# NinV/Background-Debiased-Video-CIL

Measured on AMD Instinct MI355X. Metric: clips/sec fwd+bwd TSM-R50 8x224^2 bs32/GPU, higher is better.
Workload: dtype f32; 1 GPU; TSM-ResNet50 fwd+bwd+SGD step, synthetic 32x8x3x224x224 clips per GPU, 101 classes, SimpleLinear+CrossEntropyLoss, dropout 0.5, random-init weights; fp32 tensors, accumulators and results; conv products: fp32 via 3xbf16 split, 6 MFMA products, fp32 accumulate (dropped terms <= 2^-24 relative); conv_arith=bf16x3, clips_per_gpu=32, global_batch=32, parallelism=dp1

## Files before the change

background-debiased-video-cil_amd/_lib.py:

```python
from __future__ import annotations

import ctypes
import os
from ctypes import POINTER, Structure, c_char_p, c_float, c_int, c_int32, c_int64, c_size_t, c_uint16, c_uint64, c_void_p

_HERE = os.path.dirname(os.path.abspath(__file__))
_OVERRIDE = os.environ.get('BDVCIL_LIB_PATH')
LIB_PATH = _OVERRIDE or os.path.join(_HERE, 'csrc', 'libbdvcil_hip.so')
ABI_VERSION = 32

_lib = None


class ConvGeom(Structure):
    _fields_ = [(n, c_int32) for n in
                ('N', 'H', 'W', 'Cin', 'Ho', 'Wo', 'Cout', 'R', 'S', 'stride', 'pad', 'T', 'fold', 'pad_w', 'Rt', 'st_t', 'act_dtype')]

    def key(self):
        return tuple(getattr(self, n) for n, _ in self._fields_)


P = c_void_p
_F3 = c_float * 3


class ConvAffine(Structure):
    _fields_ = [('scale', c_void_p), ('shift', c_void_p), ('residual', c_void_p), ('relu', c_int32)]


class BnStatFuse(Structure):
    _fields_ = [('y', c_void_p), ('relu_mask', c_void_p), ('mean', c_void_p), ('invstd', c_void_p), ('partial', c_void_p),
                ('relu_scale', c_void_p), ('relu_shift', c_void_p)]

class JpegInfo(Structure):
    _fields_ = [('width', c_int32), ('height', c_int32), ('ncomp', c_int32), ('h', c_int32 * 3), ('v', c_int32 * 3),
                ('blocks_w', c_int32 * 3), ('blocks_h', c_int32 * 3), ('down_w', c_int32 * 3), ('down_h', c_int32 * 3),
                ('qt', (c_uint16 * 64) * 3), ('coef_offset', c_int64 * 3), ('coef_count', c_int64)]

    def geometry_key(self):
        return (self.width, self.height, self.ncomp, tuple(self.h), tuple(self.v))


SIGNATURES = {
    'bdv_last_error': (c_char_p, []),
    'bdv_abi_version': (c_int, []),
    'bdv_source_hash': (c_char_p, []),
    'bdv_conv_workspace_bytes': (c_size_t, [POINTER(ConvGeom), c_int]),
    'bdv_conv_fprop_stat_rows': (c_int, [POINTER(ConvGeom)]),
    'bdv_conv_fprop': (c_int, [P, P, P, POINTER(ConvGeom), P, POINTER(ConvAffine), P, c_size_t, P]),
    'bdv_conv_fprop_x3': (c_int, [P, P, P, POINTER(ConvGeom), P, POINTER(ConvAffine), P, c_size_t, P]),
    'bdv_conv_dgrad_stat_rows': (c_int, [POINTER(ConvGeom)]),
    'bdv_conv_dgrad': (c_int, [P, P, P, P, P, POINTER(ConvGeom), POINTER(BnStatFuse), P, c_size_t, P]),
    'bdv_conv_dgrad_x3': (c_int, [P, P, P, P, P, P, POINTER(ConvGeom), POINTER(BnStatFuse), P, c_size_t, P]),
    'bdv_conv_weight_planes_bytes': (c_size_t, [POINTER(ConvGeom)]),
    'bdv_conv_split_weights': (c_int, [P, POINTER(ConvGeom), P, P, P]),
    'bdv_conv_fprop_pre_ok': (c_int, [POINTER(ConvGeom)]),
    'bdv_conv_fprop_pre_stat_rows': (c_int, [POINTER(ConvGeom)]),
    'bdv_conv_wgrad_pre_ok': (c_int, [POINTER(ConvGeom)]),
    'bdv_conv_debug_force_tile': (c_int, [c_int]),
    'bdv_conv_uses_planes': (c_int, [POINTER(ConvGeom), c_int, c_int]),
    'bdv_conv_kernel_name': (c_int, [POINTER(ConvGeom), c_int, c_int, c_char_p, c_size_t]),
    'bdv_conv_fprop_pl_stat_rows': (c_int, [POINTER(ConvGeom), c_int]),
    'bdv_conv_dgrad_pl_stat_rows': (c_int, [POINTER(ConvGeom), c_int]),
    'bdv_conv_fprop_pl': (c_int, [P, P, P, P, POINTER(ConvGeom), P, POINTER(ConvAffine), P, c_size_t, c_int, P, P, P]),
    'bdv_conv_dgrad_pl': (c_int, [P, P, P, P, P, P, POINTER(ConvGeom), POINTER(BnStatFuse), P, c_size_t, c_int, P]),
    'bdv_conv_wgrad': (c_int, [P, P, P, c_float, POINTER(ConvGeom), P, c_size_t, P]),
    'bdv_conv_wgrad_splits': (c_int, [POINTER(ConvGeom)]),
    'bdv_conv_wgrad_partial': (c_int, [P, P, POINTER(ConvGeom), P, c_size_t, P]),
    'bdv_conv_wgrad_partial_x3': (c_int, [P, P, POINTER(ConvGeom), P, c_size_t, P]),
    'bdv_conv_wgrad_pl_splits': (c_int, [POINTER(ConvGeom)]),
    'bdv_conv_wgrad_partial_pl': (c_int, [P, P, POINTER(ConvGeom), P, c_size_t, c_int, P, P, P]),
    'bdv_wgrad_reduce_batched': (c_int, [P, P, P, P, c_int, c_float, P]),
    'bdv_bn_workspace_bytes': (c_size_t, [c_int64, c_int]),
    'bdv_bn_train_stats': (c_int, [P, c_int64, c_int, P, P, c_float, c_float, P, P, P, P, P, P, P, c_size_t, P]),
    'bdv_bn_train_finalize': (c_int, [P, c_int, c_int64, c_int, P, P, c_float, c_float, P, P, P, P, P, P, P]),
    'bdv_bn_eval_params': (c_int, [c_int, P, P, P, P, c_float, P, P, P]),
    'bdv_bn_apply': (c_int, [P, P, P, P, P, P, P, P, c_int64, c_int, c_int, c_int, P]),
    'bdv_bn_backward': (c_int, [P, P, P, P, P, P, P, P, P, c_float, c_int64, c_int, c_int, P, c_int, P, P, P, c_size_t, c_int, P]),
    'bdv_bn_finalize_scratch_bytes': (c_size_t, [c_int]),
    'bdv_bn_finalize_splits': (c_int, [c_int, c_int]),
    'bdv_bn_train_finalize_split': (c_int, [P, c_int, c_int64, c_int, P, P, c_float, c_float, P, P, P, P, P, P, c_int, P, c_size_t, P]),
    'bdv_bn_backward_split': (c_int, [P, P, P, P, P, P, P, P, P, c_float, c_int64, c_int, c_int, P, c_int, P, P, P, c_size_t, c_int,
                                      c_int, P, c_size_t, P]),
    'bdv_bn_pair_workspace_bytes': (c_size_t, [c_int64, c_int]),
    'bdv_bn_backward_pair': (c_int, [P, P, P, P, P, P, P, c_int, P, P, P, P, P, P, P, P, P, P, c_int64, c_int, P, c_size_t, c_int, c_int,
                                     P, c_size_t, P]),
    'bdv_bn_eval_backward': (c_int, [P, P, P, P, P, P, P, P, P, P, P, c_float, c_int64, c_int, P, c_size_t, c_int, c_int, P, c_size_t, P]),
    'bdv_bn_backward_maxpool_split': (c_int, [P, P, P, P, P, P, P, P, P, P, c_float, c_int, c_int, c_int, c_int, P, c_size_t, c_int,
                                              c_int, P, c_size_t, P]),
    'bdv_bn_backward_maxpool': (c_int, [P, P, P, P, P, P, P, P, P, P, c_float, c_int, c_int, c_int, c_int, P, c_size_t, c_int, P]),
    'bdv_relu_bwd': (c_int, [P, P, P, P, c_int64, c_int, P]),
    'bdv_add': (c_int, [P, P, P, c_int64, c_int, P]),
    'bdv_nchw3_to_nhwc4': (c_int, [P, P, c_int, c_int, c_int, P]),
    'bdv_maxpool_fwd': (c_int, [P, P, P, c_int, c_int, c_int, c_int, c_int, P]),
    'bdv_maxpool_bwd': (c_int, [P, P, P, c_int, c_int, c_int, c_int, c_int, P]),
    'bdv_maxpool_t2_fwd': (c_int, [P, P, P, c_int64, c_int64, P]),
    'bdv_maxpool_t2_bwd': (c_int, [P, P, P, c_int64, c_int64, P]),
    'bdv_bn_relu_maxpool_fwd': (c_int, [P, P, P, P, P, P, c_int, c_int, c_int, c_int, c_int, P]),
    'bdv_avgpool_fwd': (c_int, [P, P, c_int, c_int, c_int, c_int, P]),
    'bdv_avgpool_bwd': (c_int, [P, P, c_int, c_int, c_int, c_int, P]),
    'bdv_bgmix_normalize_u8': (c_int, [P, P, c_int, P, c_float, _F3, _F3, _F3, P, P, c_int, c_int, c_int, c_int, P]),
    'bdv_bg_resize_crop_u8': (c_int, [P, c_int, c_int, c_int, c_int, c_int, P, P, c_int, c_int, P, P]),
    'bdv_resize_linear_u8': (c_int, [P, c_int, c_int, c_int, P, c_int, P, P, c_int, c_int, P]),
    'bdv_jpeg_parse': (c_int, [P, c_size_t, POINTER(JpegInfo)]),
    'bdv_jpeg_entropy_decode': (c_int, [P, c_size_t, POINTER(JpegInfo), P]),
    'bdv_jpeg_entropy_decode_batch': (c_int, [P, P, c_int, POINTER(JpegInfo), P, P, c_int]),
    'bdv_jpeg_workspace_bytes': (c_size_t, [POINTER(JpegInfo), c_int]),
    'bdv_jpeg_reconstruct_u8': (c_int, [P, P, POINTER(JpegInfo), c_int, P, c_size_t, P, P]),
    'bdv_temporal_median_u8': (c_int, [P, c_int64, P, P, P, P, c_int, c_int, c_int, P, P]),
    'bdv_jpeg_encode_info': (c_int, [c_int, c_int, c_int, POINTER(JpegInfo)]),
    'bdv_jpeg_forward_u8': (c_int, [P, c_int, c_int, c_int, c_int, P, P]),
    'bdv_jpeg_encode_bound': (c_size_t, [c_int, c_int]),
    'bdv_jpeg_entropy_encode': (c_int, [P, c_int, c_int, c_int, P, c_size_t, P]),
    'bdv_jpeg_entropy_encode_batch': (c_int, [P, c_int, c_int, c_int, c_int, P, c_size_t, P, c_int]),
    'bdv_crop_normalize_u8': (c_int, [P, P, c_int, c_int, c_int, _F3, _F3, P, P, c_int, c_int, c_int, c_int, P]),
    'bdv_actor_cut_mix_u8': (c_int, [P, c_int, c_int, c_int, P, c_int, c_int, c_int, P, P, c_int64, c_int, c_int, c_int, c_int, _F3, _F3, P,
                                     c_int, P, P]),
    'bdv_lsc_fwd': (c_int, [P, P, P, P, P, P, c_int, c_int, c_int, c_int, P]),
    'bdv_lsc_bwd': (c_int, [P, P, P, P, P, P, P, P, c_float, P, c_int, c_int, c_int, c_int, P]),
    'bdv_linear_fwd': (c_int, [P, P, P, P, c_int, c_int, c_int, P]),
    'bdv_linear_bwd': (c_int, [P, P, P, P, P, P, c_float, c_int, c_int, c_int, P]),
    'bdv_consensus_fwd': (c_int, [P, P, c_int, c_int, c_int, P]),
    'bdv_consensus_bwd': (c_int, [P, P, c_int, c_int, c_int, P]),
    'bdv_dropout': (c_int, [P, P, c_int64, c_float, c_uint64, P]),
    'bdv_lsc_loss': (c_int, [P, P, P, c_float, c_int, P, P, P, P, c_int, c_int, P]),
    'bdv_softce_loss': (c_int, [P, P, P, P, P, c_int, c_int, P]),
    'bdv_icarl_targets': (c_int, [P, P, c_int, P, P, c_int, c_int, P]),
    'bdv_acm_targets': (c_int, [P, P, P, c_float, P, c_int, c_int, P]),
    'bdv_softmax_mean': (c_int, [P, P, c_int, c_int, c_int, c_int, P]),
    'bdv_topk_acc': (c_int, [P, P, P, c_int, c_int, P]),
    'bdv_repr_from_features': (c_int, [P, P, P, c_int, c_int, c_int, c_int, P]),
    'bdv_nme_workspace_bytes': (c_size_t, [c_int, c_int]),
    'bdv_nme_classify': (c_int, [P, P, P, P, c_int, c_int, c_int, c_int, P, c_size_t, P]),
    'bdv_class_means': (c_int, [P, P, P, c_int, c_int, c_int, P]),
    'bdv_herding_workspace_bytes': (c_size_t, [c_int, c_int]),
    'bdv_herding_select': (c_int, [P, c_int, c_int, c_int, c_int, P, P, P, P, c_size_t, P]),
    'bdv_randaug_workspace_bytes': (c_size_t, [c_int, c_int, c_int, c_int]),
    'bdv_randaug_apply': (c_int, [P, P, P, P, c_int, c_int, c_int, c_int, P, c_size_t, P]),
    'bdv_reduce_workspace_bytes': (c_size_t, []),
    'bdv_kd_mse_fwd': (c_int, [P, P, P, c_int64, P, c_size_t, c_int, P]),
    'bdv_kd_mse_bwd': (c_int, [P, P, P, c_float, P, c_int64, c_int, P]),
    'bdv_multi_sqnorm': (c_int, [P, P, c_int, P, P, c_size_t, P]),
    'bdv_clip_coef': (c_int, [P, c_float, c_float, P, P]),
    'bdv_multi_sgd': (c_int, [P, P, P, P, P, P, c_int, c_float, c_float, P, P]),
}


class HipExtensionError(RuntimeError):
# ... 47 lines not shown
```

background-debiased-video-cil_amd/csrc/conv_mfma.hip:

```cpp
#include <stdlib.h>
#include "common.h"

#ifdef BDV_STAMPS
__device__ unsigned long long* g_stamp_buf = nullptr;
__device__ int g_stamp_cap = 0;
#define BDV_STAMP(slot)                                                                                                          \
  do {                                                                                                                           \
    if (threadIdx.x == 0 && g_stamp_buf != nullptr && (int)(blockIdx.x + gridDim.x * blockIdx.y) < g_stamp_cap) {                 \
      unsigned long long* q_ = g_stamp_buf + (size_t)(blockIdx.x + gridDim.x * blockIdx.y) * 8;                                  \
      if ((slot) == 4) asm volatile("s_waitcnt vmcnt(0)" ::: "memory");                                                          \
      q_[slot] = __builtin_amdgcn_s_memtime();                                                                                   \
      if ((slot) == 0) { q_[5] = __builtin_amdgcn_s_memrealtime(); q_[7] = __builtin_amdgcn_s_getreg((4 << 0) | (0 << 6) | (31 << 11)); } \
      if ((slot) == 4) q_[6] = __builtin_amdgcn_s_memrealtime();                                                                 \
    }                                                                                                                            \
  } while (0)
#else
#define BDV_STAMP(slot) do { } while (0)
#endif

namespace {

constexpr int BK = 32;

struct Geom {
// ... 43 lines not shown
}

__device__ __forceinline__ void fast_divmod(int m, int d, float rcp, int& q, int& r) {
  q = (int)((float)m * rcp);
  r = m - q * d;
  if (r < 0) {
    r += d;
    --q;
  }
  if (r >= d) {
    r -= d;
    ++q;
  }
}

template <int LDA, int LDB, int TM, int TN, int MS, int NS, bool SWA, bool SWB>
__device__ __forceinline__ void mma_stage(const float* __restrict__ As, const float* __restrict__ Bs,
                                          f32x16 (&acc)[TM][TN], int wm0, int wn0, int lane) {
  const int r = lane & 31, h = lane >> 5;
  const float* apv[SWA ? 8 : 1];
  const float* bpv[SWB ? 8 : 1];
#pragma unroll
  for (int c = 0; c < (SWA ? 8 : 1); ++c) apv[c] = As + h * LDA + wm0 + (r ^ (4 * c));
#pragma unroll
  for (int c = 0; c < (SWB ? 8 : 1); ++c) bpv[c] = Bs + h * LDB + wn0 + (r ^ (4 * c));
  auto ap = [&](int s, int i) { return apv[SWA ? ((s >> 1) & 7) : 0][2 * s * LDA + MS * i]; };
  auto bp = [&](int s, int j) { return bpv[SWB ? ((s >> 1) & 7) : 0][2 * s * LDB + NS * j]; };
  float a[2][TM], b[2][TN];
#pragma unroll
  for (int i = 0; i < TM; ++i) a[0][i] = ap(0, i);
#pragma unroll
  for (int j = 0; j < TN; ++j) b[0][j] = bp(0, j);
#pragma unroll
  for (int s = 0; s < BK / 2; ++s) {
    const int cur = s & 1, nxt = cur ^ 1;
    if (s + 1 < BK / 2) {
#pragma unroll
      for (int i = 0; i < TM; ++i) a[nxt][i] = ap(s + 1, i);
#pragma unroll
      for (int j = 0; j < TN; ++j) b[nxt][j] = bp(s + 1, j);
    }
#pragma unroll
    for (int i = 0; i < TM; ++i)
#pragma unroll
      for (int j = 0; j < TN; ++j)
        acc[i][j] = __builtin_amdgcn_mfma_f32_32x32x2f32(a[cur][i], b[cur][j], acc[i][j], 0, 0, 0);
    __builtin_amdgcn_sched_group_barrier(0x100, TM + TN, 0);
    __builtin_amdgcn_sched_group_barrier(0x008, TM * TN, 0);
  }
}

__device__ __forceinline__ int shift_class(int c, int fold) {
  return (fold > 0) ? (c < fold ? 1 : (c < 2 * fold ? -1 : 0)) : 0;
}

template <int LD, int PASSES>
__device__ __forceinline__ void store_transposed(float* __restrict__ dst, const float4 (&v)[PASSES], int tid) {
  const int row = tid >> 3, kg = tid & 7;
#pragma unroll
  for (int p = 0; p < PASSES; ++p) {
    float* d = dst + (4 * kg) * LD + ((row + 32 * p) ^ (4 * kg));
    d[0] = v[p].x;
    d[LD] = v[p].y;
    d[2 * LD] = v[p].z;
    d[3 * LD] = v[p].w;
  }
}

template <int LD, int COLS, int PASSES>
__device__ __forceinline__ void store_direct(float* __restrict__ dst, const float4 (&v)[PASSES], int tid) {
  constexpr int V = COLS / 4;
#pragma unroll
  for (int p = 0; p < PASSES; ++p) {
    const int idx = tid + 256 * p;
    const int krow = idx / V, c4 = idx - krow * V;
    *reinterpret_cast<float4*>(dst + krow * LD + 4 * c4) = v[p];
  }
}

__device__ __forceinline__ int acc_row(int reg, int lane) { return (reg & 3) + 8 * (reg >> 2) + 4 * (lane >> 5); }

struct Work {
  int dp_tiles, rem_tiles, split;
};

__device__ __forceinline__ int xcd_remap(int b, int n) {
  const int q = n >> 3, r = n & 7, x = b & 7, j = b >> 3;
  return (x < r ? x * (q + 1) : r * (q + 1) + (x - r) * q) + j;
}

struct WorkItem {
  int tile, kb, ke, pslot;
};

__device__ __forceinline__ WorkItem get_work(int b, const Work& wk, int nk) {
  WorkItem it;
  if (b < wk.dp_tiles) {
    it.tile = xcd_remap(b, wk.dp_tiles);
    it.kb = 0;
    it.ke = nk;
    it.pslot = -1;
  } else {
    const int rem = b - wk.dp_tiles;
    const int rt = rem / wk.split, sl = rem - rt * wk.split;
    it.tile = wk.dp_tiles + rt;
    it.kb = (int)(((long long)sl * nk) / wk.split);
    it.ke = (int)(((long long)(sl + 1) * nk) / wk.split);
    it.pslot = wk.split > 1 ? rem : -1;
  }
  return it;
}

template <int TM, int TN, int NT = 256>
__device__ __forceinline__ void store_partial(float* __restrict__ slab, int pslot, const f32x16 (&acc)[TM][TN], int tid) {
  float* base = slab + (size_t)pslot * (TM * TN * 16) * NT + tid;
#pragma unroll
  for (int i = 0; i < TM; ++i)
#pragma unroll
    for (int j = 0; j < TN; ++j)
#pragma unroll
      for (int e = 0; e < 16; ++e) base[(size_t)((i * TN + j) * 16 + e) * NT] = acc[i][j][e];
}

template <int TM, int TN>
__device__ __forceinline__ void zero_acc(f32x16 (&acc)[TM][TN]) {
#pragma unroll
  for (int i = 0; i < TM; ++i)
#pragma unroll
    for (int j = 0; j < TN; ++j)
#pragma unroll
      for (int e = 0; e < 16; ++e) acc[i][j][e] = 0.f;
}

__device__ __forceinline__ void fprop_store(float* __restrict__ y, const Geom& g, int row, int col, float v) {
  if (row < g.M) y[(size_t)row * g.Cout + col] = v;
}

struct BnStat {
  const void* y;
  const uint32_t* mask;
  const float* mean;
  const float* invstd;
  float* partial;
  int MT;
  const float* rscale;
  const float* rshift;
};

struct StatAcc {
  float4 s1, s2, mu, is;
  __device__ __forceinline__ void init(const BnStat& st, int col) {
    s1 = s2 = make_float4(0.f, 0.f, 0.f, 0.f);
    mu = *reinterpret_cast<const float4*>(st.mean + col);
    is = *reinterpret_cast<const float4*>(st.invstd + col);
  }
  __device__ __forceinline__ static unsigned sign_bits(const BnStat& st, int col, const float4 yv) {
    const float4 rsc = *reinterpret_cast<const float4*>(st.rscale + col), rsh = *reinterpret_cast<const float4*>(st.rshift + col);
    return (fmaf(yv.x, rsc.x, rsh.x) > 0.f ? 1u : 0u) | (fmaf(yv.y, rsc.y, rsh.y) > 0.f ? 2u : 0u) |
           (fmaf(yv.z, rsc.z, rsh.z) > 0.f ? 4u : 0u) | (fmaf(yv.w, rsc.w, rsh.w) > 0.f ? 8u : 0u);
  }
  __device__ __forceinline__ void accumulate(const float4 v, const float4 yv) {
    s1.x += v.x; s1.y += v.y; s1.z += v.z; s1.w += v.w;
    s2.x += v.x * ((yv.x - mu.x) * is.x);
    s2.y += v.y * ((yv.y - mu.y) * is.y);
    s2.z += v.z * ((yv.z - mu.z) * is.z);
    s2.w += v.w * ((yv.w - mu.w) * is.w);
  }
};

template <int BN, int NT = 256>
__device__ __forceinline__ void stat_flush(const StatAcc& a, const BnStat& st, float* __restrict__ smem, int Cin, int mt, int nt,
                                           int tid) {
  constexpr int V = BN / 4, G = NT / V;
  __syncthreads();
  const int grp = tid / V, c4 = tid - grp * V;
  *reinterpret_cast<float4*>(smem + grp * BN + 4 * c4) = a.s1;
  *reinterpret_cast<float4*>(smem + (G + grp) * BN + 4 * c4) = a.s2;
  __syncthreads();
  if (tid < BN) {
    float x = 0.f, y = 0.f;
#pragma unroll
    for (int k = 0; k < G; ++k) {
      x += smem[k * BN + tid];
      y += smem[(G + k) * BN + tid];
    }
    st.partial[(size_t)mt * Cin + nt * BN + tid] = x;
    st.partial[((size_t)st.MT + mt) * Cin + nt * BN + tid] = y;
  }
}

template <int BM, int BN, int WM, int WN, class F>
__device__ __forceinline__ void staged_epilogue(const f32x16 (&acc)[BM / WM / 32][BN / WN / 32], float* __restrict__ smem, int tid,
                                                F&& emit) {
  constexpr int TM = BM / WM / 32, TN = BN / WN / 32;
  constexpr int NT = 64 * WM * WN;
  constexpr int V = BN / 4;
  constexpr int PER = WM * 32 * V / NT;
  const int lane = tid & 63, wave = tid >> 6;
  const int wm = wave / WN, wn0 = (wave % WN) * 32;
#pragma unroll
  for (int i = 0; i < TM; ++i) {
    __syncthreads();
#pragma unroll
    for (int j = 0; j < TN; ++j)
#pragma unroll
      for (int e = 0; e < 16; ++e) smem[(wm * 32 + acc_row(e, lane)) * BN + wn0 + 32 * WN * j + (lane & 31)] = acc[i][j][e];
    __syncthreads();
#pragma unroll
    for (int q = 0; q < PER; ++q) {
      const int idx = tid + NT * q;
      const int lr = idx / V, c4 = idx - lr * V;
      const float4 v = *reinterpret_cast<const float4*>(smem + lr * BN + 4 * c4);
      emit(32 * WM * i + lr, 4 * c4, v);
    }
// ... 636 lines not shown
  f32x16 acc[TM][TN];
  zero_acc<TM, TN>(acc);
  const int nk = (g.Ktot + BK - 1) / BK;
  load(0);
  for (int kt = 0; kt < nk; ++kt) {
    __syncthreads();
    store_transposed<LDA, AP>(As, ra, tid);
    store_transposed<LDB, BP>(Bs, rb, tid);
    __syncthreads();
    if (kt + 1 < nk) load(kt + 1);
    mma_stage<LDA, LDB, TM, TN, 32 * WM, 32 * WN, true, true>(As, Bs, acc, wm0, wn0, lane);
  }
  fprop_epilogue<BM, BN, WM, WN>(acc, smem, y, g, epi, mt, nt, tid);
}

template <int BM, int BN, int WM, int WN>
__global__ __launch_bounds__(256, 2) void conv_fprop_c4_x3_kernel(const float* __restrict__ x, const float* __restrict__ w,
                                                                   float* __restrict__ y, Geom g, int NT, FpropEpi epi) {
  constexpr int TM = BM / WM / 32, TN = BN / WN / 32;
  constexpr int AP = BM / 32, BP = BN / 32;
  static_assert(3 * (BM + BN) * X3_LDK * 2 >= WM * 32 * BN * 4, "the epilogue stages a tile pass in the same LDS");
  __shared__ __attribute__((aligned(16))) unsigned short smem16[3 * (BM + BN) * X3_LDK];
  unsigned short* const As = smem16;
  unsigned short* const Bs = smem16 + 3 * BM * X3_LDK;
  float* const smem = reinterpret_cast<float*>(smem16);
  const int tile = xcd_remap(blockIdx.x, epi.MT * NT);
  const int mt = tile / NT, nt = tile - mt * NT;
  const int tid = threadIdx.x;
  const int lane = tid & 63, wave = tid >> 6;
  const int wm0 = (wave / WN) * 32, wn0 = (wave % WN) * 32;
  const int arow = tid >> 3, kg = tid & 7;
  const int HoWo = g.Ho * g.Wo;
  const int RS = g.R * g.S, RST = RS * g.Rt;
  const int Tin = g.T * g.st_t, pad_t = g.Rt / 2;
  const __amdgpu_buffer_rsrc_t xr = __builtin_amdgcn_make_buffer_rsrc((void*)x, 0, g.N * g.st_t * g.H * g.W * 16, 0x00020000);
  const __amdgpu_buffer_rsrc_t wr = __builtin_amdgcn_make_buffer_rsrc((void*)w, 0, g.Cout * g.Ktot * 4, 0x00020000);

  int a_base[AP], a_hi0[AP], a_wi0[AP], a_t0[AP];
#pragma unroll
  for (int p = 0; p < AP; ++p) {
    const int m = mt * BM + arow + 32 * p;
    const bool ok = m < g.M;
    const int mm = ok ? m : 0;
    const int n = mm / HoWo;
    const int rem = mm - n * HoWo;
    const int ho = rem / g.Wo, wo = rem - ho * g.Wo;
    a_hi0[p] = ok ? ho * g.stride - g.pad : -(1 << 20);
    a_wi0[p] = wo * g.stride - g.pad_w;
    a_t0[p] = (n % g.T) * g.st_t - pad_t;
    a_base[p] = (((n * g.st_t - pad_t) * g.H + ho * g.stride - g.pad) * g.W + wo * g.stride - g.pad_w) * 16;
  }
  float4 ra[AP], rb[BP];
  auto load = [&](int kt) {
    const int tap = kt * (BK / 4) + kg;
    int dt, rs, r, s;
    fast_divmod(tap, RS, g.rcp_RS, dt, rs);
    fast_divmod(rs, g.S, g.rcp_S, r, s);
    const bool kv = tap < RST;
#pragma unroll
    for (int p = 0; p < AP; ++p) {
      const bool v = kv && (unsigned)(a_hi0[p] + r) < (unsigned)g.H && (unsigned)(a_wi0[p] + s) < (unsigned)g.W &&
                     (unsigned)(a_t0[p] + dt) < (unsigned)Tin;
      ra[p] = buf_load16(xr, (a_base[p] + ((dt * g.H + r) * g.W + s) * 16) | (v ? 0 : kOOB), 0);
    }
#pragma unroll
    for (int p = 0; p < BP; ++p)
      rb[p] = buf_load16(wr, (((nt * BN + arow + 32 * p) * g.Ktot + tap * 4) * 4) | (kv ? 0 : kOOB), 0);
  };
  f32x16 acc[TM][TN];
  zero_acc<TM, TN>(acc);
  const int nk = (g.Ktot + BK - 1) / BK;
  load(0);
  for (int kt = 0; kt < nk; ++kt) {
    __syncthreads();
    store_split3<BM, AP>(As, ra, tid);
    store_split3<BN, BP>(Bs, rb, tid);
    __syncthreads();
    if (kt + 1 < nk) load(kt + 1);
    mma_stage_x3<TM, TN, 32 * WM, 32 * WN, BM, BN>(As, Bs, acc, wm0, wn0, lane);
  }
  fprop_epilogue<BM, BN, WM, WN>(acc, smem, y, g, epi, mt, nt, tid);
}

template <int BM, int BN, int WM, int WN>
__global__ __launch_bounds__(64 * WM * WN) void conv_fprop_fixup_kernel(const float* __restrict__ slab, float* __restrict__ y, Geom g,
                                                                int NT, Work wk, FpropEpi epi) {
  constexpr int TM = BM / WM / 32, TN = BN / WN / 32;
  constexpr int NACC = TM * TN * 16;
  constexpr int NTHR = 64 * WM * WN;
  __shared__ __attribute__((aligned(16))) float smem[WM * 32 * BN];
  const int rt = blockIdx.x, tile = wk.dp_tiles + rt;
  const int mt = tile / NT, nt = tile - mt * NT;
  const int tid = threadIdx.x;
  f32x16 acc[TM][TN];
  zero_acc<TM, TN>(acc);
  for (int sl = 0; sl < wk.split; ++sl) {
    const float* src = slab + (size_t)(rt * wk.split + sl) * NACC * NTHR + tid;
#pragma unroll
    for (int i = 0; i < TM; ++i)
#pragma unroll
      for (int j = 0; j < TN; ++j)
#pragma unroll
        for (int e = 0; e < 16; ++e) acc[i][j][e] += src[(size_t)((i * TN + j) * 16 + e) * NTHR];
  }
  fprop_epilogue<BM, BN, WM, WN>(acc, smem, y, g, epi, mt, nt, tid);
}

template <int BM, int BN, int WM, int WN>
__global__ __launch_bounds__(256, 3) void conv_dgrad_kernel(const float* __restrict__ dy, const float* __restrict__ w,
                                                          float* __restrict__ dx, const float* __restrict__ add_src,
                                                          const uint32_t* __restrict__ add_mask, Geom g, int NT, Work wk,
                                                          float* __restrict__ slab, BnStat stat) {
  constexpr int LDA = BM, LDB = BN;
  constexpr int TM = BM / WM / 32, TN = BN / WN / 32;
  constexpr int AP = BM / 32, BP = BN / 32;
  constexpr int BV = BN / 4;
  constexpr int AOFF = (BK * LDA + 3) & ~3;
  constexpr int SMEM = (AOFF + BK * LDB) > (WM * 32 * BN) ? (AOFF + BK * LDB) : (WM * 32 * BN);
  __shared__ __attribute__((aligned(16))) float smem[SMEM];
  float* const As = smem;
  float* const Bs = smem + AOFF;

  const int st = g.stride;
  const int ph = blockIdx.y / st, pw = blockIdx.y - ph * st;
  const int Hc = (g.H - ph + st - 1) / st, Wc = (g.W - pw + st - 1) / st;
  const int Mc = g.N * Hc * Wc;
  const int MT = (Mc + BM - 1) / BM;
  const int r0 = (ph + g.pad) % st, s0 = (pw + g.pad_w) % st;
  const int nr = r0 < g.R ? (g.R - r0 + st - 1) / st : 0;
  const int ns = s0 < g.S ? (g.S - s0 + st - 1) / st : 0;
  const int bh = (ph + g.pad - r0) / st, bw = (pw + g.pad_w - s0) / st;
  const int ntap = nr * ns;
  const int nk = ntap * g.Cout / BK;

  int mt, nt;
  WorkItem it;
  if (st == 1) {
    it = get_work(blockIdx.x, wk, nk);
    mt = it.tile / NT;
    nt = it.tile - mt * NT;
  } else {
    const int id = blockIdx.x;
    const int xcd = id & 7, jj = id >> 3;
    mt = (jj / NT) * 8 + xcd;
    nt = jj % NT;
    if (mt >= MT) return;
    it.tile = 0;
    it.kb = 0;
    it.ke = nk;
    it.pslot = -1;
  }

  const int tid = threadIdx.x;
  const int lane = tid & 63, wave = tid >> 6;
  const int wm0 = (wave / WN) * 32, wn0 = (wave % WN) * 32;
  const int arow = tid >> 3, kg = tid & 7;
  const int HcWc = Hc * Wc;
  const int RS = g.R * g.S;
  const __amdgpu_buffer_rsrc_t yr = __builtin_amdgcn_make_buffer_rsrc((void*)dy, 0, g.N * g.Ho * g.Wo * g.Cout * 4, 0x00020000);
  const __amdgpu_buffer_rsrc_t wr = __builtin_amdgcn_make_buffer_rsrc((void*)w, 0, g.Cout * RS * g.Cin * 4, 0x00020000);

  int a_base[AP], a_h[AP], a_w[AP];
#pragma unroll
  for (int p = 0; p < AP; ++p) {
    const int m = mt * BM + arow + 32 * p;
    const bool ok = m < Mc;
    const int mm = ok ? m : 0;
    const int n = mm / HcWc;
    const int rem = mm - n * HcWc;
    const int hc = rem / Wc, wc = rem - hc * Wc;
    a_h[p] = ok ? hc + bh : -(1 << 20);
    a_w[p] = wc + bw;
    a_base[p] = ((n * g.Ho + hc + bh) * g.Wo + wc + bw) * g.Cout * 4 + 16 * kg;
  }
  int b_base[BP];
#pragma unroll
  for (int p = 0; p < BP; ++p) {
    const int idx = tid + 256 * p;
    const int krow = idx / BV, c4 = idx - krow * BV;
    b_base[p] = (krow * RS * g.Cin + nt * BN + 4 * c4) * 4;
  }

  int chunk = ntap > 0 ? it.kb / ntap : 0, ir, is;
  {
    const int ct = ntap > 0 ? it.kb - chunk * ntap : 0;
    ir = ns > 0 ? ct / ns : 0;
// ... 115 lines not shown
    const int rem = mm - n * HcWc;
    const int hc = rem / Wc, wc = rem - hc * Wc;
    a_h[p] = ok ? hc + bh : -(1 << 20);
    a_w[p] = wc + bw;
    a_base[p] = ((n * g.Ho + hc + bh) * g.Wo + wc + bw) * g.Cout * 4 + 16 * kg;
  }
  int b_base[BP];
#pragma unroll
  for (int p = 0; p < BP; ++p) b_base[p] = ((nt * BN + arow + 32 * p) * g.Cout + 4 * kg) * 4;

  int chunk = ntap > 0 ? it.kb / ntap : 0, ir, is;
  {
    const int ct = ntap > 0 ? it.kb - chunk * ntap : 0;
    ir = ns > 0 ? ct / ns : 0;
    is = ct - ir * ns;
  }

  float4 ra[AP], rb[BP];
  u32x4 rbp[BPRE ? 3 * BQ : 1];
  auto load = [&]() {
    const int tap = (r0 + ir * st) * g.S + (s0 + is * st);
    const int koff_a = (chunk * BK - (ir * g.Wo + is) * g.Cout) * 4;
    const int koff_b = (tap * g.Cin * g.Cout + chunk * BK) * 4;
#pragma unroll
    for (int p = 0; p < AP; ++p) {
      const bool v = (unsigned)(a_h[p] - ir) < (unsigned)g.Ho && (unsigned)(a_w[p] - is) < (unsigned)g.Wo;
      ra[p] = buf_load16(yr, (a_base[p] + koff_a) | (v ? 0 : kOOB), 0);
    }
    if (BPRE) {
#pragma unroll
      for (int pl = 0; pl < 3; ++pl)
#pragma unroll
        for (int q = 0; q < BQ; ++q)
          rbp[pl * BQ + q] = __builtin_amdgcn_raw_buffer_load_b128(wr, (nt * BN + brow + 64 * q) * 64 + 16 * bc + pl * plane_bytes,
                                                                   (tap * nchunk + chunk) * g.Cin * 64, 0);
    } else {
#pragma unroll
      for (int p = 0; p < BP; ++p) rb[p] = buf_load16(wr, b_base[p], koff_b);
    }
    is += 1;
    const int w1 = (is == ns) ? 1 : 0;
    is = w1 ? 0 : is;
    ir += w1;
    const int w2 = (ir == nr) ? 1 : 0;
    ir = w2 ? 0 : ir;
    chunk += w2;
  };

  f32x16 acc[TM][TN];
  zero_acc<TM, TN>(acc);

  if (it.ke > it.kb) {
    load();
    for (int kt = it.kb; kt < it.ke; ++kt) {
      __syncthreads();
      store_split3<BM, AP>(As, ra, tid);
      if (BPRE) {
#pragma unroll
        for (int pl = 0; pl < 3; ++pl)
#pragma unroll
          for (int q = 0; q < BQ; ++q) *reinterpret_cast<u32x4*>(Bs + (pl * BN + brow + 64 * q) * X3_LDK + 8 * bc) = rbp[pl * BQ + q];
      } else {
        store_split3<BN, BP>(Bs, rb, tid);
      }
      __syncthreads();
      if (kt + 1 < it.ke) load();
      mma_stage_x3<TM, TN, 32 * WM, 32 * WN, BM, BN>(As, Bs, acc, wm0, wn0, lane);
    }
  }
  if (it.pslot >= 0) {
    store_partial<TM, TN>(slab, it.pslot, acc, tid);
    return;
  }

  dgrad_epilogue<BM, BN, WM, WN, true, 4, true>(acc, smem, tid, dx, add_src, add_mask, g, mt, nt, Mc, stat, [&](int mrow) {
    if (st == 1) return mrow;
    const int n = mrow / HcWc;
    const int rem = mrow - n * HcWc;
    const int hc = rem / Wc;
    return (n * g.H + hc * st + ph) * g.W + (rem - hc * Wc) * st + pw;
  });
}

template <int BM, int BN, int WM, int WN>
__global__ __launch_bounds__(64 * WM * WN) void conv_dgrad_fixup_kernel(const float* __restrict__ slab, float* __restrict__ dx,
                                                                const float* __restrict__ add_src,
                                                                const uint32_t* __restrict__ add_mask, Geom g, int NT, Work wk,
                                                                BnStat stat) {
  constexpr int TM = BM / WM / 32, TN = BN / WN / 32;
  constexpr int NACC = TM * TN * 16;
  constexpr int NTHR = 64 * WM * WN;
  __shared__ __attribute__((aligned(16))) float smem[WM * 32 * BN];
  const int rt = blockIdx.x, tile = wk.dp_tiles + rt;
  const int mt = tile / NT, nt = tile - mt * NT;
  const int tid = threadIdx.x;
  f32x16 acc[TM][TN];
  zero_acc<TM, TN>(acc);
  for (int sl = 0; sl < wk.split; ++sl) {
    const float* src = slab + (size_t)(rt * wk.split + sl) * NACC * NTHR + tid;
#pragma unroll
    for (int i = 0; i < TM; ++i)
#pragma unroll
      for (int j = 0; j < TN; ++j)
#pragma unroll
        for (int e = 0; e < 16; ++e) acc[i][j][e] += src[(size_t)((i * TN + j) * 16 + e) * NTHR];
  }
  dgrad_epilogue<BM, BN, WM, WN>(acc, smem, tid, dx, add_src, add_mask, g, mt, nt, g.M, stat, [](int mrow) { return mrow; });
}

template <int BM, int BN, int WM, int WN, bool C4, bool INCR>
__global__ __launch_bounds__(256, 3) void conv_wgrad_kernel(const float* __restrict__ dy, const float* __restrict__ x,
                                                          float* __restrict__ slab, Geom g, int MTw, int NTw,
                                                          int kt_per_split) {
  constexpr int LDA = BM, LDB = BN;
  constexpr int TM = BM / WM / 32, TN = BN / WN / 32;
  constexpr int AP = BM / 32, BP = BN / 32;
  constexpr int AV = BM / 4, BV = BN / 4;
  __shared__ __attribute__((aligned(16))) float smem[BK * (LDA + LDB)];
  float* const As = smem;
  float* const Bs = smem + BK * LDA;

  const int tiles = MTw * NTw;
  const int wi = xcd_remap(blockIdx.x, gridDim.x);
  const int split = wi / tiles;
  const int tile = wi - split * tiles;
  const int mt = tile % MTw, nt = tile / MTw;
  const int tid = threadIdx.x;
  const int lane = tid & 63, wave = tid >> 6;
  const int wm0 = (wave / WN) * 32, wn0 = (wave % WN) * 32;
  const int HoWo = g.Ho * g.Wo;
  const int frame_bytes = g.H * g.W * g.Cin * 4;
  const __amdgpu_buffer_rsrc_t xr = __builtin_amdgcn_make_buffer_rsrc((void*)x, 0, g.N * frame_bytes, 0x00020000);
  const __amdgpu_buffer_rsrc_t yr = __builtin_amdgcn_make_buffer_rsrc((void*)dy, 0, g.M * g.Cout * 4, 0x00020000);

  int a_off[AP];
#pragma unroll
  for (int p = 0; p < AP; ++p) {
    const int idx = tid + 256 * p;
    const int krow = idx / AV, c4 = idx - krow * AV;
    a_off[p] = (krow * g.Cout + mt * BM + 4 * c4) * 4;
  }
  int b_krow[BP], b_off[BP], b_r[BP], b_s[BP], b_cls[BP];
  bool b_cok[BP];
#pragma unroll
  for (int p = 0; p < BP; ++p) {
    const int idx = tid + 256 * p;
    const int krow = idx / BV, c4 = idx - krow * BV;
    b_krow[p] = krow;
    int tap, ci;
    if (C4) {
      const int ncol = nt * BN + 4 * c4;
      tap = ncol / g.Cin;
      ci = ncol - tap * g.Cin;
      b_cok[p] = ncol < g.Ktot;
    } else {
      const int per_tap = g.Cin / BN;
      tap = nt / per_tap;
      ci = (nt - tap * per_tap) * BN + 4 * c4;
      b_cok[p] = true;
    }
    b_r[p] = tap / g.S - g.pad;
    b_s[p] = tap % g.S - g.pad_w;
    b_cls[p] = shift_class(ci, g.fold);
    b_off[p] = ((b_r[p] * g.W + b_s[p]) * g.Cin + ci) * 4 + b_cls[p] * frame_bytes;
  }

  const int kt_begin = split * kt_per_split;
  const int nkt_all = (g.M + BK - 1) / BK;
  const int kt_end = min(kt_begin + kt_per_split, nkt_all);

  const int st = g.stride;
  const int d_ho = BK / g.Wo, d_wo = BK - d_ho * g.Wo;
  const int wrap_w = g.Wo * st, wrap_h = g.Ho * st;
  const int px = g.Cin * 4;
  const int inc0 = (d_ho * st * g.W + d_wo * st) * px;
  const int inc1 = (st * g.W - wrap_w) * px;
  const int inc2 = (g.H * g.W - wrap_h * g.W) * px;
  int s_hi[BP], s_wi[BP], s_t[BP], s_off[BP];
  if (INCR) {
#pragma unroll
    for (int p = 0; p < BP; ++p) {
      const int m = split * kt_per_split * BK + b_krow[p];
      const int n = m / HoWo;
      const int rem = m - n * HoWo;
      const int ho = rem / g.Wo, wo = rem - ho * g.Wo;
      s_hi[p] = ho * st;
      s_wi[p] = wo * st;
      s_t[p] = n % g.T;
// ... 372 lines not shown
  const int tx = threadIdx.x & 31, ty = threadIdx.x >> 5;
  const size_t plane = (size_t)Cout * RS * Cin;
#pragma unroll
  for (int p = 0; p < 4; ++p) {
    const int co_l = ty + 8 * p;
    const float a = w[((size_t)(co0 + co_l) * RS + tap) * Cin + ci0 + tx];
    const __bf16 hi = (__bf16)a;
    const float r1 = a - (float)hi;
    const __bf16 mid = (__bf16)r1;
    const __bf16 lo = (__bf16)(r1 - (float)mid);
    const unsigned short h16 = __builtin_bit_cast(unsigned short, hi), m16 = __builtin_bit_cast(unsigned short, mid),
                         l16 = __builtin_bit_cast(unsigned short, lo);
    if (F != nullptr) {
      const size_t o = (((size_t)(ci0 >> 5) * RS + tap) * Cout + co0 + co_l) * 32 + tx;
      F[o] = h16;
      F[plane + o] = m16;
      F[2 * plane + o] = l16;
    }
    tile[0][co_l][tx] = h16;
    tile[1][co_l][tx] = m16;
    tile[2][co_l][tx] = l16;
  }
  if (D == nullptr) return;
  __syncthreads();
#pragma unroll
  for (int p = 0; p < 4; ++p) {
    const int ci_l = ty + 8 * p;
    const size_t o = (((size_t)tap * (Cout >> 5) + (co0 >> 5)) * Cin + ci0 + ci_l) * 32 + tx;
    D[o] = tile[0][tx][ci_l];
    D[plane + o] = tile[1][tx][ci_l];
    D[2 * plane + o] = tile[2][tx][ci_l];
  }
}

using PlSet0 = std::integral_constant<int, 0>;
using PlSet1 = std::integral_constant<int, 1>;
template <typename LoadF, typename StoreF, typename MmaF>
__device__ __forceinline__ void pl_pipeline2(int n, LoadF&& load, StoreF&& store, MmaF&& mma, bool late = false) {
  load(PlSet0{});
  store(0, PlSet0{});
  if (n > 1) load(PlSet1{});
  if (n > 2) load(PlSet0{});
  __syncthreads();
  BDV_STAMP(1);
  int i = 0;
  if (late) {
    for (; i + 4 < n; i += 2) {
      store(1, PlSet1{});
      load(PlSet1{});
      mma(0);
      __syncthreads();
      store(0, PlSet0{});
      load(PlSet0{});
      mma(1);
      __syncthreads();
    }
  } else {
    for (; i + 4 < n; i += 2) {
      mma(0);
      store(1, PlSet1{});
      load(PlSet1{});
      __syncthreads();
      mma(1);
      store(0, PlSet0{});
      load(PlSet0{});
      __syncthreads();
    }
  }
  for (; i < n; i += 2) {
    mma(0);
    if (i + 1 < n) store(1, PlSet1{});
    if (i + 3 < n) load(PlSet1{});
    __syncthreads();
    if (i + 1 >= n) break;
    mma(1);
    if (i + 2 < n) store(0, PlSet0{});
    if (i + 4 < n) load(PlSet0{});
    __syncthreads();
  }
}

constexpr int pl_waves_per_simd(int waves, int np, bool fits128) { return np == 1 && waves == 8 && fits128 ? 4 : waves == 4 ? 2 : waves / 4; }

template <int BM, int BN, int WM, int WN, int NBUF, int NP = 3, bool PRE = false, int ES = 4>
__global__ __launch_bounds__(64 * WM * WN, pl_waves_per_simd(WM * WN, NP, BN == 64 || (BM == 128 && BN == 256))) void conv_fprop_pl_kernel(const void* __restrict__ x,
                                                                                      const unsigned short* __restrict__ wp,
                                                                                      void* __restrict__ y, Geom g, int NT, Work wk,
                                                                                      float* __restrict__ slab, FpropEpi epi) {
  constexpr int NTHR = 64 * WM * WN;
  constexpr int TM = BM / WM / 32, TN = BN / WN / 32;
  constexpr int KG = ES == 2 ? 4 : 8;
  constexpr int AP = BM * KG / NTHR;
  constexpr int BPP = (BN * 4 + NTHR - 1) / NTHR;
  constexpr int PA = BM * 64, PB = BN * 64, STAGE = NP * (PA + PB);
  constexpr int SMEM = NBUF * STAGE >= WM * 32 * BN * 4 ? NBUF * STAGE : WM * 32 * BN * 4;
  static_assert(AP >= 1 && SMEM <= 160 * 1024, "tile / epilogue staging do not fit");
  __shared__ __attribute__((aligned(16))) unsigned char smem_b[SMEM];
  float* const smem = reinterpret_cast<float*>(smem_b);

  BDV_STAMP(0);
  const int nk = g.Ktot / BK;
  const WorkItem it = get_work(blockIdx.x, wk, nk);
  const int mt = it.tile / NT, nt = it.tile - mt * NT;

  const int tid = threadIdx.x;
  const int lane = tid & 63, wave = tid >> 6;
  const int wm = wave / WN, wn = wave % WN;
  const int arow = tid / KG, kg = tid % KG;
  const int brow = tid >> 2, bc = tid & 3;
  const int HoWo = g.Ho * g.Wo;
  static_assert(ES == 4 || (NP == 1 && !PRE), "bf16 storage: single-product arithmetic only");
  const int frame_bytes = g.H * g.W * g.Cin * ES;
  const int plane_bytes = g.Cout * g.Ktot * 2;

  const __amdgpu_buffer_rsrc_t xr = __builtin_amdgcn_make_buffer_rsrc((void*)x, 0, g.N * frame_bytes, 0x00020000);
  const __amdgpu_buffer_rsrc_t wr = __builtin_amdgcn_make_buffer_rsrc((void*)wp, 0, 3 * plane_bytes, 0x00020000);

  int a_base[AP], a_t[AP], a_hi0[AP], a_wi0[AP];
#pragma unroll
  for (int p = 0; p < AP; ++p) {
    const int m = mt * BM + arow + (NTHR / KG) * p;
    const bool ok = m < g.M;
    int n, rem, ho, wo;
    fast_divmod(ok ? m : 0, HoWo, g.rcp_HoWo, n, rem);
    fast_divmod(rem, g.Wo, g.rcp_Wo, ho, wo);
    a_t[p] = n % g.T;
    a_hi0[p] = ok ? ho * g.stride - g.pad : -(1 << 20);
    a_wi0[p] = wo * g.stride - g.pad_w;
    a_base[p] = ((n * g.H + ho * g.stride - g.pad) * g.W + wo * g.stride - g.pad_w) * g.Cin * ES + 16 * kg;
  }
  int b_base[BPP];
  const bool b_active = BN * 4 >= NTHR || tid < BN * 4;
#pragma unroll
  for (int q = 0; q < BPP; ++q) b_base[q] = b_active ? (nt * BN + brow + (NTHR / 4) * q) * 64 + 16 * bc : kOOB;

  const int RS = g.R * g.S;
  int chunk = it.kb / RS, r, s, kt_w = it.kb;
  {
    const int tap = it.kb - chunk * RS;
    r = tap / g.S;
    s = tap - r * g.S;
  }

  constexpr int NSET = NBUF;
  float4 ra[NSET][AP];
  u32x4 rb[NSET][NP * BPP];
  float4 psc[PRE ? NSET : 1], psh[PRE ? NSET : 1];
  unsigned pvalid[PRE ? NSET : 1];
  auto load = [&](auto set) __attribute__((always_inline)) {
    constexpr int SET = decltype(set)::value;
    if constexpr (PRE) {
      psc[SET] = *reinterpret_cast<const float4*>(epi.pre_scale + chunk * BK + 4 * kg);
      psh[SET] = *reinterpret_cast<const float4*>(epi.pre_shift + chunk * BK + 4 * kg);
      pvalid[SET] = 0u;
    }
    const int cls = shift_class(chunk * BK + (BK / KG) * kg, g.fold);
    const int koff_a = ((r * g.W + s) * g.Cin + chunk * BK) * ES;
    const int koff_b = kt_w * g.Cout * 64;
#pragma unroll
    for (int p = 0; p < AP; ++p) {
      const bool v = (unsigned)(a_hi0[p] + r) < (unsigned)g.H && (unsigned)(a_wi0[p] + s) < (unsigned)g.W &&
                     (unsigned)(a_t[p] + cls) < (unsigned)g.T;
      ra[SET][p] = buf_load16(xr, (a_base[p] + koff_a + cls * frame_bytes) | (v ? 0 : kOOB), 0);
      if constexpr (PRE) pvalid[SET] |= (v ? 1u : 0u) << p;
    }
#pragma unroll
    for (int pl = 0; pl < NP; ++pl)
#pragma unroll
      for (int q = 0; q < BPP; ++q) rb[SET][pl * BPP + q] = __builtin_amdgcn_raw_buffer_load_b128(wr, b_base[q] + pl * plane_bytes, koff_b, 0);
    kt_w += 1;
    s += 1;
    const int ws_ = (s == g.S) ? 1 : 0;
    s = ws_ ? 0 : s;
    r += ws_;
    const int wr_ = (r == g.R) ? 1 : 0;
    r = wr_ ? 0 : r;
    chunk += wr_;
  };
  const int st_a = ES == 2 ? pl_off(arow, kg) : pl_off(arow, kg >> 1) + 8 * (kg & 1), st_b = pl_off(brow, bc);
  const int fa[2] = {pl_frag_off(32 * wm, 0, lane), pl_frag_off(32 * wm, 1, lane)};
  const int fb[2] = {pl_frag_off(32 * wn, 0, lane), pl_frag_off(32 * wn, 1, lane)};
  auto store = [&](int stage, auto set) __attribute__((always_inline)) {
    constexpr int SET = decltype(set)::value;
    unsigned char* const As = smem_b + stage * STAGE;
    unsigned char* const Bs = As + NP * PA;
#pragma unroll
    for (int p = 0; p < AP; ++p) {
      float4 v = ra[SET][p];
      if constexpr (PRE) {
        const bool ok = (pvalid[SET] >> p) & 1u;
        v.x = ok ? fmaxf(fmaf(v.x, psc[SET].x, psh[SET].x), 0.f) : 0.f;
        v.y = ok ? fmaxf(fmaf(v.y, psc[SET].y, psh[SET].y), 0.f) : 0.f;
        v.z = ok ? fmaxf(fmaf(v.z, psc[SET].z, psh[SET].z), 0.f) : 0.f;
        v.w = ok ? fmaxf(fmaf(v.w, psc[SET].w, psh[SET].w), 0.f) : 0.f;
      }
      if constexpr (ES == 2) *reinterpret_cast<float4*>(As + st_a + (NTHR / KG) * p * 64) = v;
      else pl_split_store_at<NP>(As + st_a + (NTHR / KG) * p * 64, PA, v);
    }
    if (b_active) {
#pragma unroll
      for (int pl = 0; pl < NP; ++pl)
#pragma unroll
        for (int q = 0; q < BPP; ++q) *reinterpret_cast<u32x4*>(Bs + st_b + (pl * PB + (NTHR / 4) * q * 64)) = rb[SET][pl * BPP + q];
    }
  };
  f32x16 acc[TM][TN];
  zero_acc<TM, TN>(acc);

  if constexpr (NBUF == 2) {
    pl_pipeline2(it.ke - it.kb, load, store, [&](int stage) __attribute__((always_inline)) {
      mma_stage_pl<BM, BN, WM, WN, NP>(smem_b + stage * STAGE, smem_b + stage * STAGE + NP * PA, acc, fa, fb);
    }, g.stagger != 0 && wave >= WM * WN / 2);
  } else {
    load(PlSet0{});
    for (int kt = it.kb; kt < it.ke; ++kt) {
      __syncthreads();
      store(0, PlSet0{});
      __syncthreads();
      if (kt == it.kb) BDV_STAMP(1);
      if (kt + 1 < it.ke) load(PlSet0{});
      mma_stage_pl<BM, BN, WM, WN, NP>(smem_b, smem_b + NP * PA, acc, fa, fb);
    }
  }
  BDV_STAMP(2);

  if (it.pslot >= 0) {
    store_partial<TM, TN, NTHR>(slab, it.pslot, acc, tid);
    return;
  }
  fprop_epilogue<BM, BN, WM, WN, ES>(acc, smem, y, g, epi, mt, nt, tid);
  BDV_STAMP(3);
  BDV_STAMP(4);
}

template <int BM, int BN, int WM, int WN, int NBUF, int NP = 3, int ES = 4>
__global__ __launch_bounds__(64 * WM * WN, BM == 64 ? 4 : pl_waves_per_simd(WM * WN, NP, BN == 64)) void conv_dgrad_pl_kernel(const void* __restrict__ dy,
                                                                                      const unsigned short* __restrict__ dp,
                                                                                      void* __restrict__ dx,
                                                                                      const void* __restrict__ add_src,
                                                                                      const uint32_t* __restrict__ add_mask, Geom g,
                                                                                      int NT, Work wk, float* __restrict__ slab,
                                                                                      BnStat stat) {
  constexpr int NTHR = 64 * WM * WN;
  constexpr int TM = BM / WM / 32, TN = BN / WN / 32;
  constexpr int KG = ES == 2 ? 4 : 8;
  constexpr int AP = BM * KG / NTHR;
  constexpr int BPP = (BN * 4 + NTHR - 1) / NTHR;
  constexpr int PA = BM * 64, PB = BN * 64, STAGE = NP * (PA + PB);
  constexpr int SMEM = NBUF * STAGE >= WM * 32 * BN * 4 ? NBUF * STAGE : WM * 32 * BN * 4;
  static_assert(AP >= 1 && SMEM <= 160 * 1024, "tile / epilogue staging do not fit");
  __shared__ __attribute__((aligned(16))) unsigned char smem_b[SMEM];
  float* const smem = reinterpret_cast<float*>(smem_b);

  BDV_STAMP(0);
  const int st = g.stride;
  const int ph = blockIdx.y / st, pw = blockIdx.y - ph * st;
  const int Hc = (g.H - ph + st - 1) / st, Wc = (g.W - pw + st - 1) / st;
  const int Mc = g.N * Hc * Wc;
  const int MT = (Mc + BM - 1) / BM;
  const int r0 = (ph + g.pad) % st, s0 = (pw + g.pad_w) % st;
  const int nr = r0 < g.R ? (g.R - r0 + st - 1) / st : 0;
  const int ns = s0 < g.S ? (g.S - s0 + st - 1) / st : 0;
  const int bh = (ph + g.pad - r0) / st, bw = (pw + g.pad_w - s0) / st;
  const int ntap = nr * ns;
  const int nk = ntap * g.Cout / BK;

  int mt, nt;
  WorkItem it;
  if (st == 1) {
    it = get_work(blockIdx.x, wk, nk);
    mt = it.tile / NT;
    nt = it.tile - mt * NT;
  } else {
    const int id = blockIdx.x;
    const int xcd = id & 7, jj = id >> 3;
    mt = (jj / NT) * 8 + xcd;
    nt = jj % NT;
    if (mt >= MT) return;
    it.tile = 0;
    it.kb = 0;
    it.ke = nk;
    it.pslot = -1;
  }

  const int tid = threadIdx.x;
  const int lane = tid & 63, wave = tid >> 6;
  const int wm = wave / WN, wn = wave % WN;
  const int arow = tid / KG, kg = tid % KG;
  const int brow = tid >> 2, bc = tid & 3;
  const int HcWc = Hc * Wc;
  const int RS = g.R * g.S;
  const int plane_bytes = g.Cout * RS * g.Cin * 2;
  const __amdgpu_buffer_rsrc_t yr = __builtin_amdgcn_make_buffer_rsrc((void*)dy, 0, g.N * g.Ho * g.Wo * g.Cout * ES, 0x00020000);
  const __amdgpu_buffer_rsrc_t wr = __builtin_amdgcn_make_buffer_rsrc((void*)dp, 0, 3 * plane_bytes, 0x00020000);

  int a_base[AP], a_h[AP], a_w[AP];
#pragma unroll
  for (int p = 0; p < AP; ++p) {
    const int m = mt * BM + arow + (NTHR / KG) * p;
    const bool ok = m < Mc;
    const int mm = ok ? m : 0;
    const int n = mm / HcWc;
    const int rem = mm - n * HcWc;
    const int hc = rem / Wc, wc = rem - hc * Wc;
    a_h[p] = ok ? hc + bh : -(1 << 20);
    a_w[p] = wc + bw;
    a_base[p] = ((n * g.Ho + hc + bh) * g.Wo + wc + bw) * g.Cout * ES + 16 * kg;
  }
  int b_base[BPP];
  const bool b_active = BN * 4 >= NTHR || tid < BN * 4;
#pragma unroll
  for (int q = 0; q < BPP; ++q) b_base[q] = b_active ? (nt * BN + brow + (NTHR / 4) * q) * 64 + 16 * bc : kOOB;

  int chunk = ntap > 0 ? it.kb / ntap : 0, ir, is;
  {
    const int ct = ntap > 0 ? it.kb - chunk * ntap : 0;
    ir = ns > 0 ? ct / ns : 0;
    is = ct - ir * ns;
  }
  const int nchunk = g.Cout / BK;

  constexpr int NSET = NBUF;
  float4 ra[NSET][AP];
  u32x4 rb[NSET][NP * BPP];
  auto load = [&](auto set) __attribute__((always_inline)) {
    constexpr int SET = decltype(set)::value;
    const int tap = (r0 + ir * st) * g.S + (s0 + is * st);
    const int koff_a = (chunk * BK - (ir * g.Wo + is) * g.Cout) * ES;
    const int koff_b = (tap * nchunk + chunk) * g.Cin * 64;
#pragma unroll
    for (int p = 0; p < AP; ++p) {
      const bool v = (unsigned)(a_h[p] - ir) < (unsigned)g.Ho && (unsigned)(a_w[p] - is) < (unsigned)g.Wo;
      ra[SET][p] = buf_load16(yr, (a_base[p] + koff_a) | (v ? 0 : kOOB), 0);
    }
#pragma unroll
    for (int pl = 0; pl < NP; ++pl)
#pragma unroll
      for (int q = 0; q < BPP; ++q) rb[SET][pl * BPP + q] = __builtin_amdgcn_raw_buffer_load_b128(wr, b_base[q] + pl * plane_bytes, koff_b, 0);
    is += 1;
    const int w1 = (is == ns) ? 1 : 0;
    is = w1 ? 0 : is;
    ir += w1;
    const int w2 = (ir == nr) ? 1 : 0;
    ir = w2 ? 0 : ir;
    chunk += w2;
  };
  const int st_a = ES == 2 ? pl_off(arow, kg) : pl_off(arow, kg >> 1) + 8 * (kg & 1), st_b = pl_off(brow, bc);
  const int fa[2] = {pl_frag_off(32 * wm, 0, lane), pl_frag_off(32 * wm, 1, lane)};
  const int fb[2] = {pl_frag_off(32 * wn, 0, lane), pl_frag_off(32 * wn, 1, lane)};
  auto store = [&](int stage, auto set) __attribute__((always_inline)) {
    constexpr int SET = decltype(set)::value;
    unsigned char* const As = smem_b + stage * STAGE;
    unsigned char* const Bs = As + NP * PA;
#pragma unroll
    for (int p = 0; p < AP; ++p) {
      if constexpr (ES == 2) *reinterpret_cast<float4*>(As + st_a + (NTHR / KG) * p * 64) = ra[SET][p];
      else pl_split_store_at<NP>(As + st_a + (NTHR / KG) * p * 64, PA, ra[SET][p]);
    }
    if (b_active) {
#pragma unroll
      for (int pl = 0; pl < NP; ++pl)
#pragma unroll
        for (int q = 0; q < BPP; ++q) *reinterpret_cast<u32x4*>(Bs + st_b + (pl * PB + (NTHR / 4) * q * 64)) = rb[SET][pl * BPP + q];
    }
  };

  f32x16 acc[TM][TN];
  zero_acc<TM, TN>(acc);

  if (it.ke > it.kb) {
    if constexpr (NBUF == 2) {
      pl_pipeline2(it.ke - it.kb, load, store, [&](int stage) __attribute__((always_inline)) {
        mma_stage_pl<BM, BN, WM, WN, NP>(smem_b + stage * STAGE, smem_b + stage * STAGE + NP * PA, acc, fa, fb);
      }, g.stagger != 0 && wave >= WM * WN / 2);
    } else {
      load(PlSet0{});
      for (int kt = it.kb; kt < it.ke; ++kt) {
        __syncthreads();
        store(0, PlSet0{});
        __syncthreads();
        if (kt == it.kb) BDV_STAMP(1);
        if (kt + 1 < it.ke) load(PlSet0{});
        mma_stage_pl<BM, BN, WM, WN, NP>(smem_b, smem_b + NP * PA, acc, fa, fb);
      }
    }
  }
  BDV_STAMP(2);
  if (it.pslot >= 0) {
    store_partial<TM, TN, NTHR>(slab, it.pslot, acc, tid);
    return;
  }
  constexpr bool EPI_PIPE = TM * TN <= 4 && NP >= 2 && BM != 64;
  dgrad_epilogue<BM, BN, WM, WN, true, ES, EPI_PIPE>(acc, smem, tid, dx, add_src, add_mask, g, mt, nt, Mc, stat, [&](int mrow) {
    if (st == 1) return mrow;
    const int n = mrow / HcWc;
    const int rem = mrow - n * HcWc;
    const int hc = rem / Wc;
    return (n * g.H + hc * st + ph) * g.W + (rem - hc * Wc) * st + pw;
  });
  BDV_STAMP(3);
  BDV_STAMP(4);
}

typedef short s16x4_t __attribute__((ext_vector_type(4)));

template <int COLS, int NP = 3, int ROWS = 32>
__device__ __forceinline__ void pl_store_rows(unsigned char* __restrict__ base, int krow, int c4, const float4 v) {
  constexpr int PITCH = 2 * COLS + 64, PLANE = ROWS * PITCH;
  if constexpr (NP == 1) {
    *reinterpret_cast<u32x2_t*>(base + krow * PITCH + 8 * c4) = bf16_hi_pairs(v);
    return;
  }
  u32x2_t hi, mid, lo;
  split3_pairs(v, hi, mid, lo);
  unsigned char* q = base + krow * PITCH + 8 * c4;
  *reinterpret_cast<u32x2_t*>(q) = hi;
  *reinterpret_cast<u32x2_t*>(q + PLANE) = mid;
  if constexpr (NP == 3) *reinterpret_cast<u32x2_t*>(q + 2 * PLANE) = lo;
}

template <int COLS>
__device__ __forceinline__ bf16x8_t pl_frag_tr(const unsigned char* __restrict__ plane, int cb, int s, int lane) {
  constexpr int PITCH = 2 * COLS + 64;
  const int h = lane >> 5, q = (lane & 15) >> 2;
  const unsigned char* a = plane + (16 * s + 8 * h + q) * PITCH + 2 * (cb + 16 * ((lane >> 4) & 1) + 4 * (lane & 3));
  typedef __attribute__((address_space(3))) s16x4_t* lds_ptr;
  const s16x4_t lo4 = __builtin_amdgcn_ds_read_tr16_b64_v4i16((lds_ptr)(a));
  const s16x4_t hi4 = __builtin_amdgcn_ds_read_tr16_b64_v4i16((lds_ptr)(a + 4 * PITCH));
  typedef short s16x8_t __attribute__((ext_vector_type(8)));
  const s16x8_t f = __builtin_shufflevector(lo4, hi4, 0, 1, 2, 3, 4, 5, 6, 7);
  return __builtin_bit_cast(bf16x8_t, f);
}

template <int BM, int BN, int WM, int WN, bool INCR, int NP = 3, bool MTAP = false, int KW = 32, int ES = 4>
__global__ __launch_bounds__(64 * WM * WN, 2) void conv_wgrad_pl_kernel(const void* __restrict__ dy, const void* __restrict__ x,
                                                                         float* __restrict__ slab, Geom g, int MTw, int NTw,
                                                                         int kt_per_split, const float* __restrict__ pre_scale,
                                                                         const float* __restrict__ pre_shift) {
  constexpr int NTHR = 64 * WM * WN;
  constexpr int TM = BM / WM / 32, TN = BN / WN / 32;
  constexpr int GV = ES == 2 ? 8 : 4;
  static_assert(TM >= 1 && TN >= 1 && (32 * (BM / GV)) % NTHR == 0 && (32 * (BN / GV)) % NTHR == 0, "tile / thread mapping");
  static_assert(ES == 4 || NP == 1, "bf16 storage: single-product arithmetic (and Cin % 8 == 0: a 16-byte unit stays inside a filter tap)");
  constexpr int AV = BM / GV, BV = BN / GV;
  static_assert(KW == 32 || KW == 16, "pixels per stage");
  constexpr int NST = 32 / KW;
  constexpr int AP = KW * AV / NTHR, BP = KW * BV / NTHR;
  static_assert(AP >= 1 && BP >= 1 && (KW * AV) % NTHR == 0 && (KW * BV) % NTHR == 0, "stage / thread mapping");
  constexpr int PITCH_A = 2 * BM + 64, PITCH_B = 2 * BN + 64;
  constexpr int PLANE_A = KW * PITCH_A, PLANE_B = KW * PITCH_B;
  constexpr int STAGE = 3 * (PLANE_A + PLANE_B);
  __shared__ __attribute__((aligned(16))) unsigned char smem_b[NST * STAGE];
  __shared__ __attribute__((aligned(16))) float pre_lds[2][BN];
  const bool pre = pre_scale != nullptr;

  const int tiles = MTw * NTw;
  const int wi = xcd_remap(blockIdx.x, gridDim.x);
  const int split = wi / tiles;
  const int tile = wi - split * tiles;
  const int mt = tile % MTw, nt = tile / MTw;
  const int tid = threadIdx.x;
  const int lane = tid & 63, wave = tid >> 6;
  const int wm = wave / WN, wn = wave % WN;
  const int HoWo = g.Ho * g.Wo;
  const int frame_bytes = g.H * g.W * g.Cin * ES;
  const __amdgpu_buffer_rsrc_t xr = __builtin_amdgcn_make_buffer_rsrc((void*)x, 0, g.N * g.st_t * frame_bytes, 0x00020000);
  const __amdgpu_buffer_rsrc_t yr = __builtin_amdgcn_make_buffer_rsrc((void*)dy, 0, g.M * g.Cout * ES, 0x00020000);

  int a_off[AP], a_krow[AP];
#pragma unroll
  for (int p = 0; p < AP; ++p) {
    const int idx = tid + NTHR * p;
    a_krow[p] = idx / AV;
    a_off[p] = (a_krow[p] * g.Cout + mt * BM + GV * (idx % AV)) * ES;
  }
  int b_krow[BP], b_off[BP], b_cls[BP], b_r[BP], b_s[BP];
// ... 293 lines not shown
  p.nk = (g.Ktot + BK - 1) / BK;
  p.seg_bytes = (size_t)(p.wide ? 64 : 32) * 256 * sizeof(float);
  if (g.Cin % BK != 0) {
    p.wk.dp_tiles = p.MT * p.NT;
    p.wk.rem_tiles = 0;
    p.wk.split = 1;
  } else {
    p.wk = (x3 && p.wide) ? plan_work(p.MT * p.NT, p.nk, 0.9, p.seg_bytes, ws_bytes, 2)
                          : plan_work(p.MT * p.NT, p.nk, p.wide ? 1.7 : 0.85, p.seg_bytes, ws_bytes);
  }
  return p;
}

FdPlan plan_dgrad(const Geom& g, size_t ws_bytes, bool x3 = false) {
  FdPlan p;
  p.wide = (g.Cin % 128) == 0;
  const int bn = p.wide ? 128 : 64;
  const int st = g.stride;
  const int Mc0 = g.N * ((g.H + st - 1) / st) * ((g.W + st - 1) / st);
  p.MT = (Mc0 + 127) / 128;
  p.NT = g.Cin / bn;
  p.nk = g.R * g.S * g.Cout / BK;
  p.seg_bytes = (size_t)(p.wide ? 64 : 32) * 256 * sizeof(float);
  if (st == 1) {
    p.wk = (x3 && p.wide) ? plan_work(p.MT * p.NT, p.nk, 0.9, p.seg_bytes, ws_bytes, 2)
                          : plan_work(p.MT * p.NT, p.nk, p.wide ? 1.7 : 0.85, p.seg_bytes, ws_bytes);
  } else {
    p.wk.dp_tiles = ((p.MT + 7) / 8) * 8 * p.NT;
    p.wk.rem_tiles = 0;
    p.wk.split = 1;
  }
  return p;
}

struct PlCfg {
  int BM, BN, nbuf;
  double iter_us;
};
constexpr int kNumPlCfg = 6;
constexpr PlCfg kPlCfg[kNumPlCfg] = {{128, 256, 2, 2.7}, {256, 128, 2, 2.7}, {256, 256, 1, 4.7}, {256, 64, 2, 1.9}, {64, 128, 1, 0.7},
                                     {128, 128, 1, 1.6}};
constexpr int pl_cfg_wm(int cfg) { return cfg == 0 || cfg == 2 || cfg == 4 || cfg == 5 ? 2 : 4; }
constexpr int pl_cfg_wn(int cfg) { return cfg == 4 || cfg == 5 ? 2 : 8 / pl_cfg_wm(cfg); }
constexpr int pl_cfg_round(int cfg) { return cfg == 5 ? 512 : 256; }

struct PlPlan {
  int cfg;
  int MT, NT, nk;
  size_t seg_bytes;
  Work wk;
  double est_us;
};

Work plan_work_pl(int tiles, int nk, double iter_us, size_t seg_bytes, size_t ws_bytes, double* est_us, int W = 256) {
  Work wk;
  const int q = tiles / W, r = tiles - q * W;
  wk.dp_tiles = tiles;
  wk.rem_tiles = 0;
  wk.split = 1;
  double best = (double)(q + (r > 0 ? 1 : 0)) * nk * iter_us;
  if (r > 0 && nk >= 4) {
    for (int sp = 2; sp <= 16 && nk / sp >= 2; ++sp) {
      const size_t need = (size_t)r * sp * seg_bytes;
      if (need > ws_bytes) break;
      const int rounds = (r * sp + W - 1) / W;
      const int per = (nk + sp - 1) / sp;
      const double cost = ((double)q * nk + (double)rounds * per) * iter_us + 8.0 + 2.0 * (double)need / 4.0e6;
      if (cost < best * 0.97) {
        best = cost;
        wk.dp_tiles = q * W;
        wk.rem_tiles = r;
        wk.split = sp;
      }
    }
  }
  *est_us = best;
  return wk;
}

int g_pl_tile_forced = -2;
int pl_tile_override() {
  if (g_pl_tile_forced == -2) g_pl_tile_forced = getenv("BDVCIL_PL_TILE") ? atoi(getenv("BDVCIL_PL_TILE")) : -1;
  return g_pl_tile_forced;
}

int pl_pick(bool dgrad, int ncols, int nk, int taps, int stride, int pieces = 3, bool shifted = false) {
  const int forced = pl_tile_override();
  if (pieces == 1) {
    const bool small_ok = dgrad && stride == 1;
    if (forced >= 0 && forced < kNumPlCfg && ncols % kPlCfg[forced].BN == 0 && (forced != 4 || small_ok)) return forced;
    static const bool np1_small = getenv("BDVCIL_NP1_SMALL_TILES") == nullptr || atoi(getenv("BDVCIL_NP1_SMALL_TILES")) != 0;
    if (np1_small && small_ok && ncols % 128 == 0) return 4;
    return ncols % 256 == 0 ? 0 : ncols % 128 == 0 ? 1 : ncols % 64 == 0 ? 3 : -1;
  }
  if (pieces == 2) {
    if (forced >= 0 && forced < kNumPlCfg && ncols % kPlCfg[forced].BN == 0 && (forced != 4 || (dgrad && stride == 1))) return forced;
    const int c = pl_pick(dgrad, ncols, nk, taps, stride, 3, shifted);
    return c >= 0 ? c : ncols % 128 == 0 ? 5 : ncols % 64 == 0 ? 3 : -1;
  }
  if (forced == kNumPlCfg) return -1;
  if (forced >= 0 && ncols % kPlCfg[forced].BN == 0 && (forced != 4 || (dgrad && stride == 1))) return forced;
  if (ncols % 64 != 0) return -1;
  if (ncols % 128 != 0) return taps > 1 ? 3 : -1;
  if (!dgrad) {
    if (ncols % 256 != 0) return nk >= 16 ? 1 : -1;
    if (nk >= 16 || nk <= 2) return 0;
    return -1;
  }
  static const bool small_tiles = getenv("BDVCIL_DGRAD_64X128") != nullptr && atoi(getenv("BDVCIL_DGRAD_64X128")) == 1;
  if (ncols % 256 != 0) return taps > 1 && stride == 1 ? 1 : (small_tiles && taps == 1 && stride == 1 && nk >= 16 ? 4 : -1);
  if (stride == 2 && taps > 1) return 0;
  if (small_tiles && shifted && taps == 1) return 4;
  if (nk <= 8 && ncols >= 1024) return -1;
  if (shifted && taps == 1 && (ncols >= 512 || nk >= 4)) return -1;
  if (ncols == 512 && nk >= 64) return 0;
  return 2;
}

PlPlan plan_pl(int cfg, int M, int ncols, int nk, size_t ws_bytes, bool ksplit_ok) {
  PlPlan p;
  p.cfg = cfg;
  p.est_us = 0.0;
  if (cfg < 0) return p;
  const PlCfg& k = kPlCfg[cfg];
  p.MT = (M + k.BM - 1) / k.BM;
  p.NT = ncols / k.BN;
  p.nk = nk;
  p.seg_bytes = (size_t)k.BM * k.BN * sizeof(float);
  if (ksplit_ok && cfg != 4) {
    p.wk = plan_work_pl(p.MT * p.NT, nk, k.iter_us, p.seg_bytes, ws_bytes, &p.est_us, pl_cfg_round(cfg));
  } else {
    p.wk.dp_tiles = p.MT * p.NT;
    p.wk.rem_tiles = 0;
    p.wk.split = 1;
    p.est_us = (double)((p.MT * p.NT + 255) / 256) * nk * k.iter_us;
  }
  return p;
}

constexpr bool r1_planes_enabled() { return true; }

bool c4_x3_enabled() {
  static const bool on = getenv("BDVCIL_C4_X3") == nullptr || atoi(getenv("BDVCIL_C4_X3")) != 0;
  return on;
}

int pl_fprop_cfg(const bdv_conv_geom* g, int pieces = 3) {
  if (g->Cin % BK != 0) return -1;
  return pl_pick(false, g->Cout, g->R * g->S * g->Cin / BK, g->R * g->S, g->stride, pieces);
}
int pl_dgrad_cfg(const bdv_conv_geom* g, int pieces = 3) {
  if (g->Cout % BK != 0) return -1;
  return pl_pick(true, g->Cin, g->R * g->S * g->Cout / BK, g->R * g->S, g->stride, pieces, g->fold > 0);
}
bool pl_fprop_ok(const bdv_conv_geom* g, int pieces = 3) { return pl_fprop_cfg(g, pieces) >= 0; }
int pl_fprop_cfg_pre(const bdv_conv_geom* g) {
  if (g->Cin % BK != 0 || g->Cout % 64 != 0) return -1;
  const int cfg = pl_fprop_cfg(g, 3);
  if (cfg >= 0) return cfg;
  return g->Cout % 256 == 0 ? 0 : g->Cout % 128 == 0 ? 1 : 3;
}
bool pl_dgrad_ok(const bdv_conv_geom* g, int pieces = 3) { return pl_dgrad_cfg(g, pieces) >= 0; }


struct WgradPlan {
  bool small;
// ... 239 lines not shown
    stat.invstd = bn_stat->invstd;
    stat.partial = bn_stat->partial;
    stat.rscale = bn_stat->relu_mask == nullptr ? bn_stat->relu_scale : nullptr;
    stat.rshift = bn_stat->relu_shift;
    stat.MT = bdv_conv_dgrad_stat_rows(gg);
    BDV_REQUIRE(stat.rscale == nullptr || w_t != nullptr || planes_d != nullptr || gg->Cin % 128 != 0,
                "bdv_conv_dgrad: a ReLU sign derived from y (relu_scale) is not compiled into the 128-wide fp32-MFMA kernel");
    if (gg->stride != 1)
      (void)hipMemsetAsync(bn_stat->partial, 0, (size_t)2 * stat.MT * gg->Cin * sizeof(float), (hipStream_t)stream);
  }
  BDV_REQUIRE(dy && w && dx, "bdv_conv_dgrad: null pointer");
  BDV_REQUIRE(bdv_aligned16(dy) && bdv_aligned16(w) && bdv_aligned16(dx) && bdv_aligned16(workspace),
              "bdv_conv_dgrad: pointers must be 16-byte aligned");
  BDV_REQUIRE(gg->Cin % 64 == 0, "bdv_conv_dgrad: Cin=%d must be a multiple of 64", gg->Cin);
  BDV_REQUIRE(add_src != nullptr || add_mask_src == nullptr, "bdv_conv_dgrad: add_mask_src without add_src");
  Geom g = make_geom(gg);
  g.M = g.N * g.H * g.W;
  g.Ktot = g.R * g.S * g.Cout;
  hipStream_t s = (hipStream_t)stream;
  const int st = g.stride;
  const bool x3 = (w_t != nullptr || planes_d != nullptr) && (g.Cin % 128) == 0;
  BDV_REQUIRE(w_t == nullptr || bdv_aligned16(w_t), "bdv_conv_dgrad_x3: w_t must be 16-byte aligned");
  const FdPlan p = plan_dgrad(g, workspace ? (workspace_bytes < kMaxSplitWorkspace ? workspace_bytes : kMaxSplitWorkspace) : 0, x3);
  const dim3 grid(p.wk.dp_tiles + p.wk.rem_tiles * p.wk.split, st * st);
  float* slab = (float*)workspace;
  if (debug_plan())
    fprintf(stderr, "[bdv plan] dgrad %dx%d Cin %d Cout %d k%d s%d: tiles %d nk %d -> dp %d rem %d split %d\n", g.H, g.W,
            g.Cin, g.Cout, g.R, g.stride, p.MT * p.NT, p.nk, p.wk.dp_tiles, p.wk.rem_tiles, p.wk.split);
  if (p.wide && x3)
    if (planes_d != nullptr)
      hipLaunchKernelGGL((conv_dgrad_x3_kernel<128, 128, 2, 2, true>), grid, dim3(256), 0, s, dy, (const float*)planes_d, dx, add_src, add_mask_src, g, p.NT, p.wk, slab, stat);
    else
      hipLaunchKernelGGL((conv_dgrad_x3_kernel<128, 128, 2, 2>), grid, dim3(256), 0, s, dy, w_t, dx, add_src, add_mask_src, g, p.NT, p.wk, slab, stat);
  else if (p.wide)
    hipLaunchKernelGGL((conv_dgrad_kernel<128, 128, 2, 2>), grid, dim3(256), 0, s, dy, w, dx, add_src, add_mask_src, g, p.NT, p.wk, slab, stat);
  else
    hipLaunchKernelGGL((conv_dgrad_kernel<128, 64, 2, 2>), grid, dim3(256), 0, s, dy, w, dx, add_src, add_mask_src, g, p.NT, p.wk, slab, stat);
  BDV_LAUNCH_CHECK("bdv_conv_dgrad");
  if (p.wk.split > 1) {
    const dim3 fg(p.wk.rem_tiles);
    if (p.wide)
      hipLaunchKernelGGL((conv_dgrad_fixup_kernel<128, 128, 2, 2>), fg, dim3(256), 0, s, (const float*)slab, dx, add_src, add_mask_src, g, p.NT, p.wk, stat);
    else
      hipLaunchKernelGGL((conv_dgrad_fixup_kernel<128, 64, 2, 2>), fg, dim3(256), 0, s, (const float*)slab, dx, add_src, add_mask_src, g, p.NT, p.wk, stat);
    BDV_LAUNCH_CHECK("bdv_conv_dgrad(fixup)");
  }
  return BDV_OK;
}
}

extern "C" int bdv_conv_dgrad(const float* dy, const float* w, float* dx, const float* add_src,
                              const uint32_t* add_mask_src, const bdv_conv_geom* gg, const bdv_bn_stat_fuse* bn_stat,
                              void* workspace, size_t workspace_bytes, void* stream) {
  return conv_dgrad_impl(dy, w, nullptr, dx, add_src, add_mask_src, gg, bn_stat, workspace, workspace_bytes, stream);
}

extern "C" int bdv_conv_dgrad_x3(const float* dy, const float* w, const float* w_t, float* dx, const float* add_src,
                                 const uint32_t* add_mask_src, const bdv_conv_geom* gg, const bdv_bn_stat_fuse* bn_stat,
                                 void* workspace, size_t workspace_bytes, void* stream) {
  BDV_REQUIRE(w_t != nullptr, "bdv_conv_dgrad_x3: w_t is null");
  return conv_dgrad_impl(dy, w, w_t, dx, add_src, add_mask_src, gg, bn_stat, workspace, workspace_bytes, stream);
}

extern "C" size_t bdv_conv_weight_planes_bytes(const bdv_conv_geom* gg) {
  if (check_geom(gg, "bdv_conv_weight_planes_bytes")) return 0;
  return (size_t)3 * gg->Cout * gg->R * gg->S * gg->Cin * sizeof(unsigned short);
}

#ifdef BDV_STAMPS
extern "C" int bdv_debug_set_stamps(void* buf, int cap_workgroups) {
  unsigned long long* p = (unsigned long long*)buf;
  if (hipMemcpyToSymbol(HIP_SYMBOL(g_stamp_buf), &p, sizeof(p)) != hipSuccess) return -1;
  if (hipMemcpyToSymbol(HIP_SYMBOL(g_stamp_cap), &cap_workgroups, sizeof(int)) != hipSuccess) return -1;
  return 0;
}
#endif

extern "C" int bdv_conv_debug_force_tile(int cfg) {
  BDV_REQUIRE(cfg >= -1 && cfg <= kNumPlCfg, "bdv_conv_debug_force_tile: cfg %d (-1 automatic, 0 = 128x256, 1 = 256x128, 2 = 256x256, 3 = 256x64, 4 = 64x128 (dgrad), 5 = 128x128 (four waves), 6 = none)", cfg);
  g_pl_tile_forced = cfg;
  return BDV_OK;
}

extern "C" int bdv_conv_kernel_name(const bdv_conv_geom* gg, int kind, int arith, char* out, size_t n) {
  if (int e = check_geom(gg, "bdv_conv_kernel_name")) return e;
  BDV_REQUIRE(out && n > 0 && kind >= 0 && kind <= 2, "bdv_conv_kernel_name: bad argument");
  const bool c4 = gg->Cin % BK != 0;
  const int pieces = arith == 2 ? 1 : arith == 3 ? 2 : 3;
  if (kind == 0) {
    const int cfg = arith ? pl_fprop_cfg(gg, pieces) : -1;
    if (cfg >= 0) {
      snprintf(out, n, "conv_fprop_pl_kernel<%d, %d, %d, %d, %d, %d>", kPlCfg[cfg].BM, kPlCfg[cfg].BN, pl_cfg_wm(cfg), pl_cfg_wn(cfg), kPlCfg[cfg].nbuf, pieces);
    } else if (c4) {
      snprintf(out, n, "conv_fprop_c4_%skernel<128, %d, 2, 2>", arith && c4_x3_enabled() ? "x3_" : "", gg->Cout % 128 == 0 ? 128 : 64);
    } else if (gg->Cout % 128 == 0 && arith) {
      snprintf(out, n, "conv_fprop_x3_kernel<128, 128, 2, 2, %s>", r1_planes_enabled() ? "true" : "false");
    } else {
      snprintf(out, n, "conv_fprop_kernel<128, %d, 2, 2>", gg->Cout % 128 == 0 ? 128 : 64);
    }
  } else if (kind == 1) {
    const int cfg = arith ? pl_dgrad_cfg(gg, pieces) : -1;
    if (cfg >= 0) {
      snprintf(out, n, "conv_dgrad_pl_kernel<%d, %d, %d, %d, %d, %d>", kPlCfg[cfg].BM, kPlCfg[cfg].BN, pl_cfg_wm(cfg), pl_cfg_wn(cfg), kPlCfg[cfg].nbuf, pieces);
    } else if (gg->Cin % 128 == 0 && arith) {
      snprintf(out, n, "conv_dgrad_x3_kernel<128, 128, 2, 2, %s>", r1_planes_enabled() ? "true" : "false");
    } else {
      snprintf(out, n, "conv_dgrad_kernel<128, %d, 2, 2>", gg->Cin % 128 == 0 ? 128 : 64);
    }
  } else {
    if (arith && pl_wgrad_ok(gg)) {
      const WgradPlPlan p = plan_wgrad_pl(gg);
      snprintf(out, n, "conv_wgrad_pl_kernel<%d, %d", p.BM, p.BN);
    } else {
      const WgradPlan p = plan_wgrad(gg);
      snprintf(out, n, "conv_wgrad_kernel<%d, %d, 2, 2", p.small ? 64 : 128, p.small ? 64 : 128);
    }
  }
  return BDV_OK;
}

extern "C" int bdv_conv_uses_planes(const bdv_conv_geom* gg, int kind, int pieces) {
  if (check_geom(gg, "bdv_conv_uses_planes")) return 0;
  if (kind == 0) return pl_fprop_ok(gg, pieces) || (pieces >= 2 && r1_planes_enabled() && gg->Cin % BK == 0 && gg->Cout % 128 == 0) ? 1 : 0;
  if (kind == 1) return pl_dgrad_ok(gg, pieces) || (pieces >= 2 && r1_planes_enabled() && gg->Cout % BK == 0 && gg->Cin % 128 == 0) ? 1 : 0;
  return 0;
}

extern "C" int bdv_conv_fprop_pl_stat_rows(const bdv_conv_geom* gg, int pieces) {
  if (check_geom(gg, "bdv_conv_fprop_pl_stat_rows")) return 0;
  if (!pl_fprop_ok(gg, pieces)) return bdv_conv_fprop_stat_rows(gg);
  const PlPlan p = plan_pl(pl_fprop_cfg(gg, pieces), gg->N * gg->Ho * gg->Wo, gg->Cout, gg->R * gg->S * gg->Cin / BK, kMaxSplitWorkspace, true);
  return p.cfg >= 0 ? p.MT : 0;
}

extern "C" int bdv_conv_fprop_pre_stat_rows(const bdv_conv_geom* gg) {
  if (check_geom(gg, "bdv_conv_fprop_pre_stat_rows")) return 0;
  const int cfg = pl_fprop_cfg_pre(gg);
  if (cfg < 0) return 0;
  const PlPlan p = plan_pl(cfg, gg->N * gg->Ho * gg->Wo, gg->Cout, gg->R * gg->S * gg->Cin / BK, kMaxSplitWorkspace, true);
  return p.MT;
}

extern "C" int bdv_conv_dgrad_pl_stat_rows(const bdv_conv_geom* gg, int pieces) {
  if (check_geom(gg, "bdv_conv_dgrad_pl_stat_rows")) return 0;
  if (!pl_dgrad_ok(gg, pieces)) return bdv_conv_dgrad_stat_rows(gg);
  const int st = gg->stride;
  const int Mc0 = gg->N * ((gg->H + st - 1) / st) * ((gg->W + st - 1) / st);
  const PlPlan p = plan_pl(pl_dgrad_cfg(gg, pieces), st == 1 ? gg->N * gg->H * gg->W : Mc0, gg->Cin, gg->R * gg->S * gg->Cout / BK,
                           kMaxSplitWorkspace, st == 1);
  return p.cfg >= 0 ? st * st * p.MT : 0;
}

extern "C" int bdv_conv_split_weights(const float* w, const bdv_conv_geom* gg, void* planes_fprop, void* planes_dgrad, void* stream) {
  if (int e = check_geom(gg, "bdv_conv_split_weights")) return e;
  BDV_REQUIRE(w && (planes_fprop || planes_dgrad), "bdv_conv_split_weights: null pointer");
  BDV_REQUIRE(gg->Cin % 32 == 0 && gg->Cout % 32 == 0, "bdv_conv_split_weights: Cin=%d and Cout=%d must be multiples of 32", gg->Cin, gg->Cout);
  BDV_REQUIRE(bdv_aligned16(w) && bdv_aligned16(planes_fprop) && bdv_aligned16(planes_dgrad), "bdv_conv_split_weights: alignment");
  const dim3 grid(gg->Cin / 32, gg->Cout / 32, gg->R * gg->S);
  hipLaunchKernelGGL(split_weights_kernel, grid, dim3(256), 0, (hipStream_t)stream, w, (unsigned short*)planes_fprop,
                     (unsigned short*)planes_dgrad, gg->Cout, gg->R * gg->S, gg->Cin);
  BDV_LAUNCH_CHECK("bdv_conv_split_weights");
  return BDV_OK;
}

extern "C" int bdv_conv_fprop_pre_ok(const bdv_conv_geom* gg) {
  if (check_geom(gg, "bdv_conv_fprop_pre_ok")) return 0;
  return pl_fprop_cfg_pre(gg) >= 0 && gg->fold == 0 ? 1 : 0;
}

extern "C" int bdv_conv_fprop_pl(const void* x, const float* w, const void* planes_fprop, void* y, const bdv_conv_geom* gg,
                                 float* bn_partial, const bdv_conv_affine* affine, void* workspace, size_t workspace_bytes,
                                 int pieces, const float* pre_scale, const float* pre_shift, void* stream) {
  if (int e = check_geom(gg, "bdv_conv_fprop_pl")) return e;
  BDV_REQUIRE(pieces >= 1 && pieces <= 3, "bdv_conv_fprop_pl: pieces = %d (3, 2 or 1)", pieces);
  const bool pre = pre_scale != nullptr;
  const bool h16 = gg->act_dtype == BDV_ACT_BF16;
  BDV_REQUIRE_ACT(gg->act_dtype, "bdv_conv_fprop_pl");
  if (h16)
    BDV_REQUIRE(pieces == 1 && !pre && planes_fprop != nullptr && pl_fprop_ok(gg, 1),
                "bdv_conv_fprop_pl: bf16 activation storage needs pieces = 1, the weight planes, Cin %% 32 == 0 and Cout %% 64 == 0 (Cin=%d Cout=%d)", gg->Cin, gg->Cout);
  if (pre) {
    BDV_REQUIRE(pre_shift != nullptr && planes_fprop != nullptr && pieces == 3 && gg->fold == 0 && pl_fprop_cfg_pre(gg) >= 0,
                "bdv_conv_fprop_pl: a producer BatchNorm in the loader needs the plane kernels (pieces 3, no temporal shift, Cin %% 32 == 0)");
    BDV_REQUIRE(bdv_aligned16(pre_scale) && bdv_aligned16(pre_shift), "bdv_conv_fprop_pl: pre_scale / pre_shift must be 16-byte aligned");
  }
  if (!pre && (planes_fprop == nullptr || !pl_fprop_ok(gg, pieces)))
    return conv_fprop_impl((const float*)x, w, (float*)y, gg, bn_partial, affine, workspace, workspace_bytes, stream, true,
                           gg->Cin % BK == 0 && r1_planes_enabled() ? planes_fprop : nullptr);
  BDV_REQUIRE(x && y, "bdv_conv_fprop_pl: null pointer");
  FpropEpi epi = {bn_partial, 0, nullptr, nullptr, nullptr, 0, pre_scale, pre_shift};
  if (affine != nullptr) {
    BDV_REQUIRE(bn_partial == nullptr, "bdv_conv_fprop_pl: batch statistics and the folded eval-mode BatchNorm exclude each other");
    BDV_REQUIRE(affine->scale && affine->shift, "bdv_conv_fprop_pl: null pointer in bdv_conv_affine");
    BDV_REQUIRE(bdv_aligned16(affine->scale) && bdv_aligned16(affine->shift) && bdv_aligned16(affine->residual),
                "bdv_conv_fprop_pl: bdv_conv_affine pointers must be 16-byte aligned");
    epi.scale = affine->scale;
    epi.shift = affine->shift;
    epi.res = affine->residual;
    epi.relu = affine->relu;
  }
  BDV_REQUIRE(bdv_aligned16(x) && bdv_aligned16(planes_fprop) && bdv_aligned16(y) && bdv_aligned16(workspace),
              "bdv_conv_fprop_pl: pointers must be 16-byte aligned");
  Geom g = make_geom(gg);
  g.M = g.N * g.Ho * g.Wo;
  g.Ktot = g.Rt * g.R * g.S * g.Cin;
  BDV_REQUIRE((int64_t)3 * g.Cout * g.Ktot * 2 < (1ll << 31), "bdv_conv_fprop_pl: weight planes exceed 2^31 bytes");
  hipStream_t s = (hipStream_t)stream;
  const PlPlan p = plan_pl(pre ? pl_fprop_cfg_pre(gg) : pl_fprop_cfg(gg, pieces), g.M, g.Cout, g.Ktot / BK, workspace ? (workspace_bytes < kMaxSplitWorkspace ? workspace_bytes : kMaxSplitWorkspace) : 0, !h16);
  BDV_REQUIRE(p.cfg >= 0, "bdv_conv_fprop_pl: no tile configuration for Cout=%d", g.Cout);
  const int blocks = p.wk.dp_tiles + p.wk.rem_tiles * p.wk.split;
  epi.MT = p.MT;
  float* slab = (float*)workspace;
  const unsigned short* wp = (const unsigned short*)planes_fprop;
  if (debug_plan())
    fprintf(stderr, "[bdv plan] fprop_pl %dx%d Cin %d Cout %d k%d s%d: cfg %d tiles %d nk %d -> dp %d rem %d split %d (est %.0f us)\n", g.H,
            g.W, g.Cin, g.Cout, g.R, g.stride, p.cfg, p.MT * p.NT, p.nk, p.wk.dp_tiles, p.wk.rem_tiles, p.wk.split, p.est_us);
#define BDV_FPROP_PL(BM_, BN_, WM_, WN_, NB_)                                                                                         \
  do {                                                                                                                                \
    if (h16)                                                                                                                          \
      hipLaunchKernelGGL((conv_fprop_pl_kernel<BM_, BN_, WM_, WN_, NB_, 1, false, 2>), dim3(blocks), dim3(64 * WM_ * WN_), 0, s, x, wp, y, \
                         g, p.NT, p.wk, slab, epi);                                                                                   \
    else if (pre)                                                                                                                     \
      hipLaunchKernelGGL((conv_fprop_pl_kernel<BM_, BN_, WM_, WN_, NB_, 3, true>), dim3(blocks), dim3(64 * WM_ * WN_), 0, s, x, wp, y,  \
                         g, p.NT, p.wk, slab, epi);                                                                                   \
    else if (pieces == 1)                                                                                                             \
      hipLaunchKernelGGL((conv_fprop_pl_kernel<BM_, BN_, WM_, WN_, NB_, 1>), dim3(blocks), dim3(64 * WM_ * WN_), 0, s, x, wp, y, g,    \
                         p.NT, p.wk, slab, epi);                                                                                      \
    else if (pieces == 2)                                                                                                             \
      hipLaunchKernelGGL((conv_fprop_pl_kernel<BM_, BN_, WM_, WN_, NB_, 2>), dim3(blocks), dim3(64 * WM_ * WN_), 0, s, x, wp, y, g,    \
                         p.NT, p.wk, slab, epi);                                                                                      \
    else                                                                                                                              \
      hipLaunchKernelGGL((conv_fprop_pl_kernel<BM_, BN_, WM_, WN_, NB_, 3>), dim3(blocks), dim3(64 * WM_ * WN_), 0, s, x, wp, y, g,    \
                         p.NT, p.wk, slab, epi);                                                                                      \
    BDV_LAUNCH_CHECK("bdv_conv_fprop_pl");                                                                                            \
    if (p.wk.split > 1) {                                                                                                             \
      hipLaunchKernelGGL((conv_fprop_fixup_kernel<BM_, BN_, WM_, WN_>), dim3(p.wk.rem_tiles), dim3(64 * WM_ * WN_), 0, s,             \
                         (const float*)slab, (float*)y, g, p.NT, p.wk, epi);                                                                  \
      BDV_LAUNCH_CHECK("bdv_conv_fprop_pl(fixup)");                                                                                   \
    }                                                                                                                                 \
  } while (0)
  if (p.cfg == 0) BDV_FPROP_PL(128, 256, 2, 4, 2);
  else if (p.cfg == 1) BDV_FPROP_PL(256, 128, 4, 2, 2);
  else if (p.cfg == 2) BDV_FPROP_PL(256, 256, 2, 4, 1);
  else if (p.cfg == 5) BDV_FPROP_PL(128, 128, 2, 2, 1);
  else BDV_FPROP_PL(256, 64, 4, 2, 2);
#undef BDV_FPROP_PL
  return BDV_OK;
}

extern "C" int bdv_conv_dgrad_pl(const void* dy, const float* w, const void* planes_dgrad, void* dx, const void* add_src,
                                 const uint32_t* add_mask_src, const bdv_conv_geom* gg, const bdv_bn_stat_fuse* bn_stat,
                                 void* workspace, size_t workspace_bytes, int pieces, void* stream) {
  if (int e = check_geom(gg, "bdv_conv_dgrad_pl")) return e;
  BDV_REQUIRE(pieces >= 1 && pieces <= 3, "bdv_conv_dgrad_pl: pieces = %d (3, 2 or 1)", pieces);
  const bool h16 = gg->act_dtype == BDV_ACT_BF16;
  BDV_REQUIRE_ACT(gg->act_dtype, "bdv_conv_dgrad_pl");
  if (h16)
    BDV_REQUIRE(pieces == 1 && planes_dgrad != nullptr && pl_dgrad_ok(gg, 1),
                "bdv_conv_dgrad_pl: bf16 activation storage needs pieces = 1, the weight planes, Cout %% 32 == 0 and Cin %% 64 == 0 (Cin=%d Cout=%d)", gg->Cin, gg->Cout);
  if (planes_dgrad == nullptr || !pl_dgrad_ok(gg, pieces))
    return conv_dgrad_impl((const float*)dy, w, nullptr, (float*)dx, (const float*)add_src, add_mask_src, gg, bn_stat, workspace, workspace_bytes, stream,
                           gg->Cout % BK == 0 && r1_planes_enabled() ? planes_dgrad : nullptr);
  BnStat stat = {nullptr, nullptr, nullptr, nullptr, nullptr, 0, nullptr, nullptr};
  if (bn_stat != nullptr) {
    BDV_REQUIRE(gg->stride == 1 || (gg->R >= gg->stride && gg->S >= gg->stride),
                "bdv_conv_dgrad_pl: fused BatchNorm statistics with stride 2 need a filter that reaches every input pixel (R, S >= 2)");
    BDV_REQUIRE(bn_stat->y && bn_stat->mean && bn_stat->invstd && bn_stat->partial, "bdv_conv_dgrad_pl: null pointer in bdv_bn_stat_fuse");
    BDV_REQUIRE(bdv_aligned16(bn_stat->y) && bdv_aligned16(bn_stat->mean) && bdv_aligned16(bn_stat->invstd) &&
                    bdv_aligned16(bn_stat->partial), "bdv_conv_dgrad_pl: bdv_bn_stat_fuse pointers must be 16-byte aligned");
    BDV_REQUIRE(bn_stat->relu_mask == nullptr || gg->Cin % 32 == 0, "bdv_conv_dgrad_pl: a ReLU mask needs Cin %% 32 == 0");
    stat.y = bn_stat->y;
    stat.mask = bn_stat->relu_mask;
    stat.mean = bn_stat->mean;
    stat.invstd = bn_stat->invstd;
    stat.partial = bn_stat->partial;
    stat.rscale = bn_stat->relu_mask == nullptr ? bn_stat->relu_scale : nullptr;
    stat.rshift = bn_stat->relu_shift;
  }
  BDV_REQUIRE(dy && dx, "bdv_conv_dgrad_pl: null pointer");
  BDV_REQUIRE(bdv_aligned16(dy) && bdv_aligned16(planes_dgrad) && bdv_aligned16(dx) && bdv_aligned16(workspace),
              "bdv_conv_dgrad_pl: pointers must be 16-byte aligned");
  BDV_REQUIRE(add_src != nullptr || add_mask_src == nullptr, "bdv_conv_dgrad_pl: add_mask_src without add_src");
  Geom g = make_geom(gg);
  g.M = g.N * g.H * g.W;
  g.Ktot = g.R * g.S * g.Cout;
  BDV_REQUIRE((int64_t)3 * g.Cin * g.Ktot * 2 < (1ll << 31), "bdv_conv_dgrad_pl: weight planes exceed 2^31 bytes");
  hipStream_t s = (hipStream_t)stream;
  const int st = g.stride;
  const int Mc0 = g.N * ((g.H + st - 1) / st) * ((g.W + st - 1) / st);
  PlPlan p = plan_pl(pl_dgrad_cfg(gg, pieces), st == 1 ? g.M : Mc0, g.Cin, g.Ktot / BK,
                     workspace ? (workspace_bytes < kMaxSplitWorkspace ? workspace_bytes : kMaxSplitWorkspace) : 0, st == 1 && !h16);
  BDV_REQUIRE(p.cfg >= 0, "bdv_conv_dgrad_pl: no tile configuration for Cin=%d", g.Cin);
  if (st != 1) p.wk.dp_tiles = ((p.MT + 7) / 8) * 8 * p.NT;
  stat.MT = st * st * p.MT;
  if (st != 1 && stat.y != nullptr)
    (void)hipMemsetAsync(stat.partial, 0, (size_t)2 * stat.MT * g.Cin * sizeof(float), s);
  const int work_items = p.wk.dp_tiles + p.wk.rem_tiles * p.wk.split;
  const dim3 grid(work_items, st * st);
  float* slab = (float*)workspace;
  const unsigned short* dp = (const unsigned short*)planes_dgrad;
  if (debug_plan())
    fprintf(stderr, "[bdv plan] dgrad_pl %dx%d Cin %d Cout %d k%d s%d: cfg %d tiles %d nk %d -> dp %d rem %d split %d (est %.0f us)\n", g.H,
            g.W, g.Cin, g.Cout, g.R, g.stride, p.cfg, p.MT * p.NT, p.nk, p.wk.dp_tiles, p.wk.rem_tiles, p.wk.split, p.est_us);
#define BDV_DGRAD_PL(BM_, BN_, WM_, WN_, NB_)                                                                                          \
  do {                                                                                                                                 \
    if (h16)                                                                                                                           \
      hipLaunchKernelGGL((conv_dgrad_pl_kernel<BM_, BN_, WM_, WN_, NB_, 1, 2>), grid, dim3(64 * WM_ * WN_), 0, s, dy, dp, dx, add_src,  \
                         add_mask_src, g, p.NT, p.wk, slab, stat);                                                                     \
    else if (pieces == 1)                                                                                                              \
      hipLaunchKernelGGL((conv_dgrad_pl_kernel<BM_, BN_, WM_, WN_, NB_, 1>), grid, dim3(64 * WM_ * WN_), 0, s, dy, dp, dx, add_src,     \
                         add_mask_src, g, p.NT, p.wk, slab, stat);                                                                     \
    else if (pieces == 2)                                                                                                              \
      hipLaunchKernelGGL((conv_dgrad_pl_kernel<BM_, BN_, WM_, WN_, NB_, 2>), grid, dim3(64 * WM_ * WN_), 0, s, dy, dp, dx, add_src,     \
                         add_mask_src, g, p.NT, p.wk, slab, stat);                                                                     \
    else                                                                                                                               \
      hipLaunchKernelGGL((conv_dgrad_pl_kernel<BM_, BN_, WM_, WN_, NB_, 3>), grid, dim3(64 * WM_ * WN_), 0, s, dy, dp, dx, add_src,     \
                         add_mask_src, g, p.NT, p.wk, slab, stat);                                                                     \
    BDV_LAUNCH_CHECK("bdv_conv_dgrad_pl");                                                                                             \
    if (p.wk.split > 1) {                                                                                                              \
      hipLaunchKernelGGL((conv_dgrad_fixup_kernel<BM_, BN_, WM_, WN_>), dim3(p.wk.rem_tiles), dim3(64 * WM_ * WN_), 0, s,              \
                         (const float*)slab, (float*)dx, (const float*)add_src, add_mask_src, g, p.NT, p.wk, stat);                                          \
      BDV_LAUNCH_CHECK("bdv_conv_dgrad_pl(fixup)");                                                                                    \
    }                                                                                                                                  \
  } while (0)
  if (p.cfg == 0) BDV_DGRAD_PL(128, 256, 2, 4, 2);
  else if (p.cfg == 1) BDV_DGRAD_PL(256, 128, 4, 2, 2);
  else if (p.cfg == 2) BDV_DGRAD_PL(256, 256, 2, 4, 1);
  else if (p.cfg == 4) BDV_DGRAD_PL(64, 128, 2, 2, 1);
  else if (p.cfg == 5) BDV_DGRAD_PL(128, 128, 2, 2, 1);
  else BDV_DGRAD_PL(256, 64, 4, 2, 2);
#undef BDV_DGRAD_PL
  return BDV_OK;
}

namespace {

int wgrad_partial(const char* who, const float* dy, const float* x, const bdv_conv_geom* gg, void* workspace, size_t workspace_bytes,
                  hipStream_t s, int* splits_out, bool x3 = false) {
  BDV_REQUIRE(gg == nullptr || gg->Rt <= 1, "%s: temporal taps (Rt=%d) need the bf16-piece plane kernel (bdv_conv_wgrad_partial_pl, BDVCIL_C4_X3)", who, gg->Rt);
  const WgradPlan p = plan_wgrad(gg);
  const size_t need = (size_t)p.splits * gg->Cout * gg->R * gg->S * gg->Cin * sizeof(float);
  if (workspace_bytes < need) {
    bdv_set_error("%s: workspace %zu < required %zu bytes", who, workspace_bytes, need);
    return BDV_EWORKSPACE;
  }
  Geom g = make_geom(gg);
  g.M = g.N * g.Ho * g.Wo;
  g.Ktot = g.Rt * g.R * g.S * g.Cin;
  float* slab = (float*)workspace;
  const dim3 grid(p.MTw * p.NTw * p.splits);
  if (debug_plan())
    fprintf(stderr, "[bdv plan] wgrad %dx%d Cin %d Cout %d k%d s%d: tiles %d -> splits %d x %d k-iters (%s)\n", gg->H, gg->W,
            gg->Cin, gg->Cout, gg->R, gg->stride, p.MTw * p.NTw, p.splits, p.kt_per_split, p.small ? "64x64" : "128x128");
  const bool incr = g.Ho * g.Wo > BK && BK / g.Wo + 1 <= g.Ho;
#define BDV_WGRAD(BMN, C4F)                                                                                                    \
  do {                                                                                                                         \
    if (incr)                                                                                                                  \
      hipLaunchKernelGGL((conv_wgrad_kernel<BMN, BMN, 2, 2, C4F, true>), grid, dim3(256), 0, s, dy, x, slab, g, p.MTw, p.NTw,   \
                         p.kt_per_split);                                                                                      \
    else                                                                                                                       \
      hipLaunchKernelGGL((conv_wgrad_kernel<BMN, BMN, 2, 2, C4F, false>), grid, dim3(256), 0, s, dy, x, slab, g, p.MTw, p.NTw,  \
                         p.kt_per_split);                                                                                      \
  } while (0)
  if (!p.small && x3) {
    if (incr)
      hipLaunchKernelGGL((conv_wgrad_x3_kernel<128, 128, 2, 2, false, true>), grid, dim3(256), 0, s, dy, x, slab, g, p.MTw, p.NTw,
                         p.kt_per_split);
    else
      hipLaunchKernelGGL((conv_wgrad_x3_kernel<128, 128, 2, 2, false, false>), grid, dim3(256), 0, s, dy, x, slab, g, p.MTw, p.NTw,
                         p.kt_per_split);
  } else if (!p.small) {
    BDV_WGRAD(128, false);
  } else if (p.c4) {
    BDV_WGRAD(64, true);
  } else {
    BDV_WGRAD(64, false);
  }
#undef BDV_WGRAD
  BDV_LAUNCH_CHECK(who);
  *splits_out = p.splits;
  return BDV_OK;
}

}

extern "C" int bdv_conv_wgrad(const float* dy, const float* x, float* dw, float beta, const bdv_conv_geom* gg,
                              void* workspace, size_t workspace_bytes, void* stream) {
  if (int e = check_geom(gg, "bdv_conv_wgrad")) return e;
  BDV_REQUIRE(dy && x && dw && workspace, "bdv_conv_wgrad: null pointer");
  BDV_REQUIRE(bdv_aligned16(dy) && bdv_aligned16(x) && bdv_aligned16(dw) && bdv_aligned16(workspace),
              "bdv_conv_wgrad: pointers must be 16-byte aligned");
  hipStream_t s = (hipStream_t)stream;
  int splits = 0;
  if (int e = wgrad_partial("bdv_conv_wgrad", dy, x, gg, workspace, workspace_bytes, s, &splits)) return e;
  const int64_t numel4 = (int64_t)gg->Cout * gg->R * gg->S * gg->Cin / 4;
  hipLaunchKernelGGL(wgrad_reduce_kernel, dim3((int)((numel4 + 63) / 64)), dim3(256), 0, s, (const float*)workspace, dw, beta, splits,
                     numel4);
  BDV_LAUNCH_CHECK("bdv_conv_wgrad(reduce)");
  return BDV_OK;
}

extern "C" int bdv_conv_wgrad_splits(const bdv_conv_geom* gg) {
  if (check_geom(gg, "bdv_conv_wgrad_splits")) return 0;
  return plan_wgrad(gg).splits;
}

extern "C" int bdv_conv_wgrad_partial(const float* dy, const float* x, const bdv_conv_geom* gg, void* slab, size_t slab_bytes,
                                      void* stream) {
  if (int e = check_geom(gg, "bdv_conv_wgrad_partial")) return e;
  BDV_REQUIRE(dy && x && slab, "bdv_conv_wgrad_partial: null pointer");
  BDV_REQUIRE(bdv_aligned16(dy) && bdv_aligned16(x) && bdv_aligned16(slab), "bdv_conv_wgrad_partial: pointers must be 16-byte aligned");
  int splits = 0;
  return wgrad_partial("bdv_conv_wgrad_partial", dy, x, gg, slab, slab_bytes, (hipStream_t)stream, &splits);
}

// ... 107 lines not shown
```

background-debiased-video-cil_amd/kernels.py:

```python
from __future__ import annotations

import ctypes
from typing import Optional, Sequence, Tuple

import torch

from ._lib import BnStatFuse, ConvAffine, ConvGeom, check, lib

_WS = {}


def _stream():
    return ctypes.c_void_p(torch.cuda.current_stream().cuda_stream)


def _p(t: Optional[torch.Tensor]):
    return ctypes.c_void_p(0 if t is None else t.data_ptr())


def _chk(t: torch.Tensor, shape: Optional[Sequence[int]] = None, dtype=torch.float32, name='tensor'):
    if not isinstance(t, torch.Tensor):
        raise TypeError(f'{name}: expected a tensor, got {type(t)}')
    if not t.is_cuda:
        raise RuntimeError(f'{name}: the HIP path needs a GPU tensor (got device {t.device}); there is no CPU fallback')
    if t.dtype != dtype:
        raise TypeError(f'{name}: dtype {t.dtype}, expected {dtype}')
    if not t.is_contiguous():
        raise ValueError(f'{name}: must be contiguous, got strides {t.stride()} for shape {tuple(t.shape)}')
    if shape is not None and tuple(t.shape) != tuple(shape):
        raise ValueError(f'{name}: shape {tuple(t.shape)}, expected {tuple(shape)}')
    return t


ACT_DTYPE = torch.float32


def _act_code(t: torch.Tensor) -> int:
    return 1 if t.dtype == torch.bfloat16 else 0


def _chk_act(t: torch.Tensor, shape=None, name='tensor', like: Optional[torch.Tensor] = None):
    if isinstance(t, torch.Tensor) and t.dtype not in (torch.float32, torch.bfloat16):
        raise TypeError(f'{name}: dtype {t.dtype}, expected torch.float32 or torch.bfloat16')
    if like is not None and isinstance(t, torch.Tensor) and t.dtype != like.dtype:
        raise TypeError(f'{name}: dtype {t.dtype} differs from the other activation operand ({like.dtype})')
    return _chk(t, shape, dtype=t.dtype if isinstance(t, torch.Tensor) else torch.float32, name=name)


def _chk_conv(t: torch.Tensor, shape, g, name):
    if isinstance(t, torch.Tensor) and t.dtype == torch.bfloat16:
        if g.act_dtype != 1:
            raise TypeError(f'{name}: bf16 tensor in an fp32 convolution call (operands of one call share the storage type)')
    elif g.act_dtype != 0:
        raise TypeError(f'{name}: dtype {getattr(t, "dtype", None)} in a bf16-storage convolution call')
    if getattr(g, 'frames_view', False):
        _chk(t, None, dtype=t.dtype, name=name)
        n = 1
        for d in shape:
            n *= d
        if t.numel() != n or t.shape[-1] != shape[-1]:
            raise ValueError(f'{name}: shape {tuple(t.shape)} is not a view of {tuple(shape)}')
        return t
    return _chk(t, shape, dtype=torch.bfloat16 if g.act_dtype == 1 else torch.float32, name=name)


def workspace(nbytes: int, device, tag='ws') -> torch.Tensor:
    key = (torch.device(device).index or 0, tag)
    cur = _WS.get(key)
    if cur is None or cur.numel() < nbytes:
        cur = torch.empty(max(int(nbytes), 1 << 20), dtype=torch.uint8, device=device)
        _WS[key] = cur
    return cur


def make_geom(N, H, W, Cin, Cout, R, S, stride, pad, T=1, fold=0, pad_w=None, rt=0, st_t=0) -> ConvGeom:
    pw = pad if pad_w is None else pad_w
    Ho = (H + 2 * pad - R) // stride + 1
    Wo = (W + 2 * pw - S) // stride + 1
    return ConvGeom(N, H, W, Cin, Ho, Wo, Cout, R, S, stride, pad, T, fold, -1 if pad_w is None else pad_w, rt, st_t)


def _in_frames(g: ConvGeom) -> int:
    return g.N * g.st_t if g.Rt > 1 else g.N


def _taps_r(g: ConvGeom) -> int:
    return g.R * g.Rt if g.Rt > 1 else g.R


def make_temporal_geom(B, T, H, W, Cin, Cout, kt) -> ConvGeom:
    g = make_geom(B, T, H * W, Cin, Cout, kt, 1, 1, kt // 2, pad_w=0)
    g.frames_view = True
    return g



WS_TAG_SUFFIX = ''


def _conv_ws(g: ConvGeom, kind: int, device, tag: str) -> torch.Tensor:
    need = lib().bdv_conv_workspace_bytes(ctypes.byref(g), kind)
    if need == 0:
        check(-1, 'bdv_conv_workspace_bytes')
    return workspace(need, device, tag + WS_TAG_SUFFIX)


import os as _os

_F32MFMA = _os.environ.get('BDVCIL_CONV_F32MFMA', '0') != '0'


def _x3_default(name):
    v = _os.environ.get(name)
    return (not _F32MFMA) if v is None else v != '0'


FPROP_X3 = _x3_default('BDVCIL_FPROP_X3')


PIECES = 3


def set_conv_arith(mode: str):
    global FPROP_X3, DGRAD_X3, WGRAD_X3, PIECES, ACT_DTYPE
    if mode not in ('bf16x3', 'f32mfma', 'bf16x2', 'bf16x1', 'bf16'):
        raise ValueError(f"set_conv_arith: unknown mode {mode!r} ('bf16x3' | 'f32mfma' | 'bf16x2' | 'bf16x1' | 'bf16')")
    prev = (FPROP_X3, DGRAD_X3, WGRAD_X3)
    FPROP_X3 = DGRAD_X3 = WGRAD_X3 = (mode != 'f32mfma')
    PIECES = 1 if mode in ('bf16x1', 'bf16') else 2 if mode == 'bf16x2' else 3
    ACT_DTYPE = torch.bfloat16 if mode == 'bf16' else torch.float32
    return prev


import weakref as _weakref

WEIGHT_EPOCH = 0
_PLANES = {}
CHECK_PLANES = _os.environ.get('BDVCIL_CHECK_PLANES', '0') != '0'


def _weight_checksum(w: torch.Tensor) -> int:
    return int(w.contiguous().view(torch.int32).to(torch.int64).sum().item())
USE_PL = _os.environ.get('BDVCIL_PL', '1') != '0'
USE_PL_WGRAD = _os.environ.get('BDVCIL_PL_WGRAD', '1') != '0'


def bump_weight_epoch(params=None):
    global WEIGHT_EPOCH
    if params is None:
        WEIGHT_EPOCH += 1
        return
    for p in params:
        ent = _PLANES.get(id(p))
        if ent is not None:
            ent[1] = None


_PLANES_PENDING = {}


def _plane_stamp(w, base):
    return (w.data_ptr(), base._version, WEIGHT_EPOCH)


def weight_planes(w: torch.Tensor, g: ConvGeom):
    if _PLANES_PENDING:
        pend = _PLANES_PENDING.get(w.device.index)
        if pend is not None:
            cur = torch.cuda.current_stream(w.device)
            if cur.cuda_stream not in pend[1]:
                cur.wait_event(pend[0])
                pend[1].add(cur.cuda_stream)
    base = w._base if w._base is not None else w
    key = id(base)
    stamp = _plane_stamp(w, base)
    ent = _PLANES.get(key)
    if ent is not None and ent[0]() is not base:
        ent = None
    nbytes = lib().bdv_conv_weight_planes_bytes(ctypes.byref(g))
    if nbytes == 0:
        check(-1, 'bdv_conv_weight_planes_bytes')
    if ent is None or ent[1] != stamp or ent[2].numel() != 2 * nbytes:
        buf = ent[2] if ent is not None and ent[2].numel() == 2 * nbytes and ent[2].device == w.device else \
            torch.empty(2 * nbytes, dtype=torch.uint8, device=w.device)
        check(lib().bdv_conv_split_weights(_p(w), ctypes.byref(g), _p(buf[:nbytes]), _p(buf[nbytes:]), _stream()),
              'bdv_conv_split_weights')
        ref = _weakref.ref(base, lambda _r, k=key: _PLANES.pop(k, None))
# ... 25 lines not shown
        st = stream if stream is not None and stream.device == device else cur
        if st != cur:
            st.wait_stream(cur)
        with torch.cuda.stream(st):
            for ent, w, base in todo:
                R, S, Cin, Cout = ent[4]
                g = make_geom(1, R, S, Cin, Cout, R, S, 1, 0, 1, 0)
                buf = ent[2]
                nbytes = buf.numel() // 2
                check(lib().bdv_conv_split_weights(_p(w), ctypes.byref(g), _p(buf[:nbytes]), _p(buf[nbytes:]), _stream()),
                      'bdv_conv_split_weights')
                ent[1] = _plane_stamp(w, base)
                if CHECK_PLANES:
                    ent[5] = _weight_checksum(w)
                n += 1
            if st != cur:
                ev = torch.cuda.Event()
                ev.record(st)
                _PLANES_PENDING[device.index] = (ev, {st.cuda_stream})
    return n


def conv_kernel_name(g: ConvGeom, kind: str, x3: Optional[bool] = None) -> str:
    k = {'fprop': 0, 'dgrad': 1, 'wgrad': 2}[kind]
    flag = (FPROP_X3, DGRAD_X3, WGRAD_X3)[k] if x3 is None else x3
    buf = ctypes.create_string_buffer(128)
    check(lib().bdv_conv_kernel_name(ctypes.byref(g), k, {3: 1, 1: 2, 2: 3}[PIECES] if flag else 0, buf, 128), 'bdv_conv_kernel_name')
    return buf.value.decode()


def conv_uses_planes(g: ConvGeom, kind: str) -> bool:
    k = {'fprop': 0, 'dgrad': 1}[kind]
    flag = (FPROP_X3, DGRAD_X3)[k]
    return bool(flag and USE_PL and lib().bdv_conv_uses_planes(ctypes.byref(g), k, PIECES))


PRE_BN_1X1_ONLY = _os.environ.get('BDVCIL_PRE_BN_3X3', '0') == '0'


def fprop_pre_ok(g: ConvGeom) -> bool:
    if PRE_BN_1X1_ONLY and (g.R != 1 or g.S != 1):
        return False
    return bool(PIECES == 3 and FPROP_X3 and WGRAD_X3 and DGRAD_X3 and USE_PL and USE_PL_WGRAD and g.fold == 0 and g.Rt <= 1
                and not getattr(g, 'frames_view', False)
                and lib().bdv_conv_fprop_pre_ok(ctypes.byref(g)) and lib().bdv_conv_wgrad_pre_ok(ctypes.byref(g)))


def conv_fprop(x: torch.Tensor, w: torch.Tensor, g: ConvGeom, out: Optional[torch.Tensor] = None,
               ws_tag: str = 'conv', bn_stats: bool = False, affine=None, x3: Optional[bool] = None, pre_bn=None):
    g.act_dtype = _act_code(x)
    _chk_conv(x, (_in_frames(g), g.H, g.W, g.Cin), g, 'x')
    _chk(w, (g.Cout, _taps_r(g), g.S, g.Cin), name='w')
    y = out if out is not None else torch.empty((g.N, g.Ho, g.Wo, g.Cout), dtype=x.dtype, device=x.device)
    _chk_conv(y, (g.N, g.Ho, g.Wo, g.Cout), g, 'y')
    ws = _conv_ws(g, 0, x.device, ws_tag)
    part = aff = None
    use_x3 = FPROP_X3 if x3 is None else x3
    use_pl = bool(use_x3 and USE_PL and lib().bdv_conv_uses_planes(ctypes.byref(g), 0, PIECES))
    if g.act_dtype == 1 and not (use_pl and PIECES == 1):
        raise ValueError("conv_fprop: bf16 tensors need set_conv_arith('bf16') and a geometry of the plane kernels (Cin % 32 == 0, Cout % 64 == 0)")
    if pre_bn is not None:
        if not (use_x3 and USE_PL and PIECES == 3 and lib().bdv_conv_fprop_pre_ok(ctypes.byref(g))):
            raise ValueError('conv_fprop: pre_bn needs the bf16-piece plane kernels for this geometry (fprop_pre_ok)')
        _chk(pre_bn[0], (g.Cin,), name='pre_scale')
        _chk(pre_bn[1], (g.Cin,), name='pre_shift')
        use_pl = True
    if bn_stats:
        if affine is not None:
            raise ValueError('conv_fprop: bn_stats and affine exclude each other')
        rows = lib().bdv_conv_fprop_pre_stat_rows(ctypes.byref(g)) if pre_bn is not None else \
            lib().bdv_conv_fprop_pl_stat_rows(ctypes.byref(g), PIECES) if use_pl else lib().bdv_conv_fprop_stat_rows(ctypes.byref(g))
        if rows <= 0:
            check(-1, 'bdv_conv_fprop_stat_rows')
        part = torch.empty((2, rows, g.Cout), dtype=torch.float32, device=x.device)
    if affine is not None:
        scale, shift, res, relu = affine
        _chk(scale, (g.Cout,), name='scale')
        _chk(shift, (g.Cout,), name='shift')
        if res is not None:
            _chk_conv(res, (g.N, g.Ho, g.Wo, g.Cout), g, 'residual')
        aff = ConvAffine(scale.data_ptr(), shift.data_ptr(), res.data_ptr() if res is not None else None, int(bool(relu)))
    if use_pl:
        planes_f, _ = weight_planes(w, g)
        check(lib().bdv_conv_fprop_pl(_p(x), _p(w), _p(planes_f), _p(y), ctypes.byref(g), _p(part),
                                      ctypes.byref(aff) if aff is not None else None, _p(ws), ws.numel(), PIECES,
                                      _p(pre_bn[0] if pre_bn is not None else None), _p(pre_bn[1] if pre_bn is not None else None),
                                      _stream()), 'bdv_conv_fprop_pl')
        return (y, part) if bn_stats else y
    fn = lib().bdv_conv_fprop_x3 if use_x3 else lib().bdv_conv_fprop
    check(fn(_p(x), _p(w), _p(y), ctypes.byref(g), _p(part), ctypes.byref(aff) if aff is not None else None,
             _p(ws), ws.numel(), _stream()), 'bdv_conv_fprop')
    return (y, part) if bn_stats else y


DGRAD_X3 = _x3_default('BDVCIL_DGRAD_X3')


def conv_dgrad(dy: torch.Tensor, w: torch.Tensor, g: ConvGeom, add_src: Optional[torch.Tensor] = None,
               add_mask_src: Optional[torch.Tensor] = None, out: Optional[torch.Tensor] = None,
               ws_tag: str = 'conv', bn_stats=None, x3: Optional[bool] = None):
    g.act_dtype = _act_code(dy)
    _chk_conv(dy, (g.N, g.Ho, g.Wo, g.Cout), g, 'dy')
    _chk(w, (g.Cout, g.R, g.S, g.Cin), name='w')
    dx = out if out is not None else torch.empty((g.N, g.H, g.W, g.Cin), dtype=dy.dtype, device=dy.device)
    _chk_conv(dx, (g.N, g.H, g.W, g.Cin), g, 'dx')
    if add_src is not None:
        _chk_conv(add_src, (g.N, g.H, g.W, g.Cin), g, 'add_src')
        if add_src.data_ptr() == dx.data_ptr() and g.fold > 0:
            raise ValueError('conv_dgrad: in-place add_src is not allowed with a temporal shift (scatter epilogue)')
    if add_mask_src is not None:
        _chk(add_mask_src, (g.N * g.H * g.W * g.Cin // 32,), dtype=torch.int32, name='add_mask_src')
    fuse = partial = None
    use_x3 = (DGRAD_X3 if x3 is None else x3) and g.Cin % 64 == 0
    use_pl = bool(use_x3 and USE_PL and lib().bdv_conv_uses_planes(ctypes.byref(g), 1, PIECES))
    if g.act_dtype == 1 and not (use_pl and PIECES == 1):
        raise ValueError("conv_dgrad: bf16 tensors need set_conv_arith('bf16') and a geometry of the plane kernels (Cout % 32 == 0, Cin % 64 == 0)")
    relu_affine = None
    if bn_stats is not None:
        if len(bn_stats) == 5:
            y, mask, mean, invstd, relu_affine = bn_stats
        else:
            y, mask, mean, invstd = bn_stats
        _chk_conv(y, (g.N, g.H, g.W, g.Cin), g, 'y')
        _chk(mean, (g.Cin,), name='mean')
        _chk(invstd, (g.Cin,), name='invstd')
        if mask is not None:
            _chk(mask, (y.numel() // 32,), dtype=torch.int32, name='relu_mask')
        rows = lib().bdv_conv_dgrad_pl_stat_rows(ctypes.byref(g), PIECES) if use_pl else lib().bdv_conv_dgrad_stat_rows(ctypes.byref(g))
        if rows <= 0:
            check(-1, 'bdv_conv_dgrad_stat_rows')
        partial = torch.empty((2, rows, g.Cin), dtype=torch.float32, device=dy.device)
        if relu_affine is not None:
            if mask is not None:
                raise ValueError('conv_dgrad: a ReLU mask and a derived ReLU sign exclude each other')
            _chk(relu_affine[0], (g.Cin,), name='relu_scale')
            _chk(relu_affine[1], (g.Cin,), name='relu_shift')
        fuse = BnStatFuse(y.data_ptr(), mask.data_ptr() if mask is not None else None, mean.data_ptr(), invstd.data_ptr(),
                          partial.data_ptr(), relu_affine[0].data_ptr() if relu_affine is not None else None,
                          relu_affine[1].data_ptr() if relu_affine is not None else None)
    ws = _conv_ws(g, 1, dy.device, ws_tag)
    if use_pl:
        _, planes_d = weight_planes(w, g)
        check(lib().bdv_conv_dgrad_pl(_p(dy), _p(w), _p(planes_d), _p(dx), _p(add_src), _p(add_mask_src), ctypes.byref(g),
                                      ctypes.byref(fuse) if fuse is not None else None, _p(ws), ws.numel(), PIECES, _stream()),
              'bdv_conv_dgrad_pl')
        return dx if bn_stats is None else (dx, partial)
    if use_x3 and g.Cin % 128 == 0:
        w_t = w.permute(1, 2, 3, 0).contiguous()
        check(lib().bdv_conv_dgrad_x3(_p(dy), _p(w), _p(w_t), _p(dx), _p(add_src), _p(add_mask_src), ctypes.byref(g),
                                      ctypes.byref(fuse) if fuse is not None else None, _p(ws), ws.numel(), _stream()),
              'bdv_conv_dgrad_x3')
        return dx if bn_stats is None else (dx, partial)
    check(lib().bdv_conv_dgrad(_p(dy), _p(w), _p(dx), _p(add_src), _p(add_mask_src), ctypes.byref(g),
                               ctypes.byref(fuse) if fuse is not None else None, _p(ws), ws.numel(), _stream()), 'bdv_conv_dgrad')
    return dx if bn_stats is None else (dx, partial)


def conv_wgrad(dy: torch.Tensor, x: torch.Tensor, g: ConvGeom, dw: Optional[torch.Tensor] = None,
               beta: float = 0.0, ws_tag: str = 'wgrad', x3: Optional[bool] = None, pre_bn=None) -> torch.Tensor:
    g.act_dtype = _act_code(dy)
    _chk_conv(dy, (g.N, g.Ho, g.Wo, g.Cout), g, 'dy')
    _chk_conv(x, (_in_frames(g), g.H, g.W, g.Cin), g, 'x')
    if dw is None:
        dw = torch.empty((g.Cout, _taps_r(g), g.S, g.Cin), dtype=torch.float32, device=dy.device)
        beta = 0.0
    _chk(dw, (g.Cout, _taps_r(g), g.S, g.Cin), name='dw')
    if WGRAD_X3 if x3 is None else x3:
        slab, _ = conv_wgrad_partial(dy, x, g, x3=True, dw=dw, pre_bn=pre_bn)
        wgrad_reduce_batched([(slab, dw)], beta=beta)
        return dw
    if pre_bn is not None:
        raise ValueError('conv_wgrad: pre_bn needs the bf16-piece plane kernel')
    ws = _conv_ws(g, 2, dy.device, ws_tag)
    check(lib().bdv_conv_wgrad(_p(dy), _p(x), _p(dw), float(beta), ctypes.byref(g), _p(ws), ws.numel(), _stream()),
          'bdv_conv_wgrad')
    return dw



def _bn_ws(M, C, device):
    return workspace(lib().bdv_bn_workspace_bytes(int(M), int(C)), device, 'bn')


_FIN_SCRATCH = {}
_FIN_SCRATCH_MIN_C = 2048


def _bn_fin_scratch(C, device):
    dev = torch.device(device)
    key = (dev.index or 0, torch.cuda.current_stream(dev).cuda_stream)
    cur = _FIN_SCRATCH.get(key)
    need = lib().bdv_bn_finalize_scratch_bytes(max(int(C), _FIN_SCRATCH_MIN_C))
    if cur is None or cur.numel() < need:
        cur = torch.zeros(need, dtype=torch.uint8, device=dev)
        _FIN_SCRATCH[key] = cur
    return cur


def bn_train_stats(y, gamma, beta, eps, momentum, running_mean, running_var):
    C = y.shape[-1]
    M = y.numel() // C
    _chk(y, name='y')
    for t, n in ((gamma, 'gamma'), (beta, 'beta')):
        _chk(t, (C,), name=n)
    if running_mean is not None:
        _chk(running_mean, (C,), name='running_mean')
        _chk(running_var, (C,), name='running_var')
    stats = torch.empty((4, C), dtype=torch.float32, device=y.device)
    ws = _bn_ws(M, C, y.device)
    check(lib().bdv_bn_train_stats(_p(y), M, C, _p(gamma), _p(beta), float(eps), float(momentum), _p(running_mean),
                                   _p(running_var), _p(stats[0]), _p(stats[1]), _p(stats[2]), _p(stats[3]), _p(ws),
                                   ws.numel(), _stream()), 'bdv_bn_train_stats')
    return stats[0], stats[1], stats[2], stats[3]


def bn_train_finalize(partial, M, gamma, beta, eps, momentum, running_mean, running_var, splits=0):
    _chk(partial, name='partial')
    _, rows, C = partial.shape
    for t, n in ((gamma, 'gamma'), (beta, 'beta')):
        _chk(t, (C,), name=n)
    if running_mean is not None:
        _chk(running_mean, (C,), name='running_mean')
        _chk(running_var, (C,), name='running_var')
    stats = torch.empty((4, C), dtype=torch.float32, device=partial.device)
    fs = _bn_fin_scratch(C, partial.device) if splits != 1 else None
    check(lib().bdv_bn_train_finalize_split(_p(partial), rows, int(M), C, _p(gamma), _p(beta), float(eps), float(momentum),
                                            _p(running_mean), _p(running_var), _p(stats[0]), _p(stats[1]), _p(stats[2]),
                                            _p(stats[3]), int(splits), _p(fs), fs.numel() if fs is not None else 0, _stream()),
# ... 740 lines not shown
```

include/bdvcil_hip.h:

```cpp
#ifndef BDVCIL_HIP_H
#define BDVCIL_HIP_H

#include <stddef.h>
#include <stdint.h>

#ifdef __cplusplus
extern "C" {
#endif

#define BDV_OK 0
#define BDV_EINVAL (-1)
#define BDV_EWORKSPACE (-2)

#define BDV_ACT_F32 0
#define BDV_ACT_BF16 1

typedef struct bdv_conv_geom {
  int32_t N;
  int32_t H, W;
  int32_t Cin;
  int32_t Ho, Wo;
  int32_t Cout;
  int32_t R, S;
  int32_t stride;
  int32_t pad;
  int32_t T;
  int32_t fold;
  int32_t pad_w;
  int32_t Rt;
  int32_t st_t;
  int32_t act_dtype;
} bdv_conv_geom;

const char* bdv_last_error(void);
int bdv_abi_version(void);
const char* bdv_source_hash(void);

size_t bdv_conv_workspace_bytes(const bdv_conv_geom* g, int kind);
int bdv_conv_fprop_stat_rows(const bdv_conv_geom* g);
typedef struct bdv_conv_affine {
  const float* scale;
  const float* shift;
  const void* residual;
  int32_t relu;
} bdv_conv_affine;
int bdv_conv_fprop(const float* x, const float* w, float* y, const bdv_conv_geom* g, float* bn_partial,
                   const bdv_conv_affine* affine, void* workspace, size_t workspace_bytes, void* stream);
int bdv_conv_fprop_x3(const float* x, const float* w, float* y, const bdv_conv_geom* g, float* bn_partial,
                      const bdv_conv_affine* affine, void* workspace, size_t workspace_bytes, void* stream);

typedef struct bdv_bn_stat_fuse {
  const void* y;
  const uint32_t* relu_mask;
  const float* mean;
  const float* invstd;
  float* partial;
  const float* relu_scale;
  const float* relu_shift;
} bdv_bn_stat_fuse;
int bdv_conv_dgrad_stat_rows(const bdv_conv_geom* g);

int bdv_conv_dgrad(const float* dy, const float* w, float* dx, const float* add_src,
                   const uint32_t* add_mask_src, const bdv_conv_geom* g, const bdv_bn_stat_fuse* bn_stat, void* workspace,
                   size_t workspace_bytes, void* stream);
int bdv_conv_dgrad_x3(const float* dy, const float* w, const float* w_t, float* dx, const float* add_src,
                      const uint32_t* add_mask_src, const bdv_conv_geom* g, const bdv_bn_stat_fuse* bn_stat, void* workspace,
                      size_t workspace_bytes, void* stream);

size_t bdv_conv_weight_planes_bytes(const bdv_conv_geom* g);
int bdv_conv_split_weights(const float* w, const bdv_conv_geom* g, void* planes_fprop, void* planes_dgrad, void* stream);
int bdv_conv_debug_force_tile(int cfg);
int bdv_conv_uses_planes(const bdv_conv_geom* g, int kind, int pieces);
int bdv_conv_kernel_name(const bdv_conv_geom* g, int kind, int arith, char* out, size_t n);
int bdv_conv_fprop_pl_stat_rows(const bdv_conv_geom* g, int pieces);
int bdv_conv_dgrad_pl_stat_rows(const bdv_conv_geom* g, int pieces);
int bdv_conv_fprop_pl(const void* x, const float* w, const void* planes_fprop, void* y, const bdv_conv_geom* g,
                      float* bn_partial, const bdv_conv_affine* affine, void* workspace, size_t workspace_bytes, int pieces,
                      const float* pre_scale, const float* pre_shift, void* stream);
int bdv_conv_fprop_pre_ok(const bdv_conv_geom* g);
int bdv_conv_fprop_pre_stat_rows(const bdv_conv_geom* g);
int bdv_conv_dgrad_pl(const void* dy, const float* w, const void* planes_dgrad, void* dx, const void* add_src,
                      const uint32_t* add_mask_src, const bdv_conv_geom* g, const bdv_bn_stat_fuse* bn_stat, void* workspace,
                      size_t workspace_bytes, int pieces, void* stream);

int bdv_conv_wgrad(const float* dy, const float* x, float* dw, float beta, const bdv_conv_geom* g, void* workspace,
                   size_t workspace_bytes, void* stream);
#define BDV_MAX_REDUCE_ITEMS 32
int bdv_conv_wgrad_splits(const bdv_conv_geom* g);
int bdv_conv_wgrad_partial(const float* dy, const float* x, const bdv_conv_geom* g, void* slab, size_t slab_bytes,
                           void* stream);
int bdv_wgrad_reduce_batched(const float* const* slabs, float* const* dws, const int* splits, const int64_t* numels, int n,
                             float beta, void* stream);
int bdv_conv_wgrad_pl_splits(const bdv_conv_geom* g);
int bdv_conv_wgrad_partial_pl(const void* dy, const void* x, const bdv_conv_geom* g, void* slab, size_t slab_bytes,
                              int pieces, const float* pre_scale, const float* pre_shift, void* stream);
int bdv_conv_wgrad_pre_ok(const bdv_conv_geom* g);
int bdv_conv_wgrad_partial_x3(const float* dy, const float* x, const bdv_conv_geom* g, void* slab, size_t slab_bytes,
                              void* stream);

size_t bdv_bn_workspace_bytes(int64_t M, int C);
int bdv_bn_train_stats(const float* y, int64_t M, int C, const float* gamma, const float* beta,
                       float eps, float momentum, float* running_mean, float* running_var,
                       float* save_mean, float* save_invstd, float* scale, float* shift,
                       void* workspace, size_t workspace_bytes, void* stream);
int bdv_bn_train_finalize(const float* partial, int rows, int64_t M, int C, const float* gamma, const float* beta,
                          float eps, float momentum, float* running_mean, float* running_var, float* save_mean,
                          float* save_invstd, float* scale, float* shift, void* stream);
int bdv_bn_eval_params(int C, const float* gamma, const float* beta, const float* running_mean,
                       const float* running_var, float eps, float* scale, float* shift, void* stream);
int bdv_bn_apply(const void* y, const float* scale, const float* shift, const void* res, const float* res_scale,
                 const float* res_shift, void* out, uint32_t* relu_mask, int64_t M, int C, int relu, int act_dtype, void* stream);
int bdv_bn_backward(const void* dout, const uint32_t* relu_mask, const void* y, const float* gamma,
                    const float* save_mean, const float* save_invstd, void* dy, float* dgamma,
                    float* dbeta, float beta_acc, int64_t M, int C, int relu, const float* stat_partial, int stat_rows,
                    const float* relu_scale, const float* relu_shift, void* workspace, size_t workspace_bytes, int act_dtype,
                    void* stream);
size_t bdv_bn_finalize_scratch_bytes(int C);
int bdv_bn_finalize_splits(int rows, int C);
int bdv_bn_train_finalize_split(const float* partial, int rows, int64_t M, int C, const float* gamma, const float* beta,
                                float eps, float momentum, float* running_mean, float* running_var, float* save_mean,
                                float* save_invstd, float* scale, float* shift, int splits, void* fin_scratch,
                                size_t fin_scratch_bytes, void* stream);
int bdv_bn_backward_split(const void* dout, const uint32_t* relu_mask, const void* y, const float* gamma,
                          const float* save_mean, const float* save_invstd, void* dy, float* dgamma,
                          float* dbeta, float beta_acc, int64_t M, int C, int relu, const float* stat_partial, int stat_rows,
                          const float* relu_scale, const float* relu_shift, void* workspace, size_t workspace_bytes, int act_dtype,
                          int splits, void* fin_scratch, size_t fin_scratch_bytes, void* stream);
size_t bdv_bn_pair_workspace_bytes(int64_t M, int C);
int bdv_bn_backward_pair(const void* dout, const uint32_t* relu_mask, const void* ya, const float* gamma_a,
                         const float* mean_a, const float* invstd_a, const float* stat_partial_a, int stat_rows_a,
                         void* dya, float* dgamma_a, float* dbeta_a, const void* yb, const float* gamma_b,
                         const float* mean_b, const float* invstd_b, void* dyb, float* dgamma_b, float* dbeta_b,
                         int64_t M, int C, void* workspace, size_t workspace_bytes, int act_dtype, int splits,
                         void* fin_scratch, size_t fin_scratch_bytes, void* stream);
int bdv_bn_eval_backward(const void* dout, const uint32_t* relu_mask, const void* relu_act, const void* y,
                         const float* scale, const float* running_mean, const float* invstd, void* dy, void* dz,
                         float* dgamma, float* dbeta, float beta_acc, int64_t M, int C, void* workspace,
                         size_t workspace_bytes, int act_dtype, int splits, void* fin_scratch, size_t fin_scratch_bytes,
                         void* stream);
int bdv_relu_bwd(const void* dout, const uint32_t* relu_mask, const void* add, void* g, int64_t numel, int act_dtype, void* stream);
int bdv_add(const void* a, const void* b, void* out, int64_t numel, int act_dtype, void* stream);

int bdv_nchw3_to_nhwc4(const float* x, float* out, int N, int H, int W, void* stream);
int bdv_maxpool_fwd(const float* x, void* out, uint8_t* idx, int N, int H, int W, int C, int out_dtype, void* stream);
int bdv_maxpool_bwd(const void* dout, const uint8_t* idx, float* dx, int N, int H, int W, int C, int dout_dtype, void* stream);
int bdv_maxpool_t2_fwd(const float* x, float* out, uint32_t* sel, int64_t frames_out, int64_t frame_elems, void* stream);
int bdv_maxpool_t2_bwd(const float* dout, const uint32_t* sel, float* dx, int64_t frames_out, int64_t frame_elems, void* stream);
int bdv_bn_backward_maxpool(const void* dpool, const uint8_t* pool_idx, const uint32_t* relu_mask, const float* y,
                            const float* gamma, const float* save_mean, const float* save_invstd, float* dy, float* dgamma,
                            float* dbeta, float beta_acc, int N, int H, int W, int C, void* workspace,
                            size_t workspace_bytes, int dpool_dtype, void* stream);
int bdv_bn_backward_maxpool_split(const void* dpool, const uint8_t* pool_idx, const uint32_t* relu_mask, const float* y,
                                  const float* gamma, const float* save_mean, const float* save_invstd, float* dy, float* dgamma,
                                  float* dbeta, float beta_acc, int N, int H, int W, int C, void* workspace,
                                  size_t workspace_bytes, int dpool_dtype, int splits, void* fin_scratch,
                                  size_t fin_scratch_bytes, void* stream);
int bdv_bn_relu_maxpool_fwd(const float* y, const float* scale, const float* shift, void* out, uint8_t* idx,
                            uint32_t* relu_mask, int N, int H, int W, int C, int out_dtype, void* stream);
int bdv_avgpool_fwd(const void* x, float* out, int N, int HW, int C, int act_dtype, void* stream);
int bdv_avgpool_bwd(const float* dout, void* dx, int N, int HW, int C, int act_dtype, void* stream);

int bdv_bgmix_normalize_u8(const uint8_t* frames, const void* bg, int bg_f32, const uint8_t* mix, float alpha,
                           const float mean[3], const float std[3], const float inv_std[3],
                           float* out_nhwc4, float* out_nchw, int B, int T, int H, int W, void* stream);
int bdv_bg_resize_crop_u8(const uint8_t* src, int B, int Hs, int Ws, int Hr, int Wr, const int32_t* top,
                          const int32_t* left, int crop_h, int crop_w, float* out, void* stream);
// ... 92 lines not shown
```

Baseline: 608.9 clips/s.

## Combine split-K partials in-kernel via last-arriver ticket instead of fixup launch

For split-K plane conv kernels (fprop and dgrad), each CTA writes its partial with buffer stores and then bumps a per-tile atomic ticket. The last CTA to arrive sums the other partials and runs the epilogue itself, so the separate fixup kernel launch is skipped. The aim is to remove a kernel launch and the extra round trip through the slab per split conv. In exchange it adds atomics, fences and block syncs, and the last arriver does serialized reduction work. Ticket buffers are allocated per stream, and an environment variable can force the old fixup path.

```diff
diff --git a/background-debiased-video-cil_amd/_lib.py b/background-debiased-video-cil_amd/_lib.py
--- a/background-debiased-video-cil_amd/_lib.py
+++ b/background-debiased-video-cil_amd/_lib.py
@@ -64,6 +64,12 @@
     'bdv_conv_dgrad_pl_stat_rows': (c_int, [POINTER(ConvGeom), c_int]),
     'bdv_conv_fprop_pl': (c_int, [P, P, P, P, POINTER(ConvGeom), P, POINTER(ConvAffine), P, c_size_t, c_int, P, P, P]),
     'bdv_conv_dgrad_pl': (c_int, [P, P, P, P, P, P, POINTER(ConvGeom), POINTER(BnStatFuse), P, c_size_t, c_int, P]),
+    'bdv_conv_ksplit_ticket_bytes': (c_size_t, []),
+    'bdv_conv_fprop_pl_tickets': (c_int, [P, P, P, P, POINTER(ConvGeom), P, POINTER(ConvAffine), P, c_size_t, c_int, P, P, P, c_size_t, P]),
+    'bdv_conv_dgrad_pl_tickets': (c_int, [P, P, P, P, P, P, POINTER(ConvGeom), POINTER(BnStatFuse), P, c_size_t, c_int, P, c_size_t, P]),
+    'bdv_conv_debug_force_fixup': (c_int, [c_int]),
+    'bdv_conv_debug_last_plan': (c_int, [POINTER(c_int)]),
+    'bdv_conv_debug_pl_plan': (c_int, [POINTER(ConvGeom), c_int, c_int, POINTER(c_int)]),
     'bdv_conv_wgrad': (c_int, [P, P, P, c_float, POINTER(ConvGeom), P, c_size_t, P]),
     'bdv_conv_wgrad_splits': (c_int, [POINTER(ConvGeom)]),
     'bdv_conv_wgrad_partial': (c_int, [P, P, POINTER(ConvGeom), P, c_size_t, P]),
diff --git a/background-debiased-video-cil_amd/csrc/conv_mfma.hip b/background-debiased-video-cil_amd/csrc/conv_mfma.hip
--- a/background-debiased-video-cil_amd/csrc/conv_mfma.hip
+++ b/background-debiased-video-cil_amd/csrc/conv_mfma.hip
@@ -149,6 +149,7 @@
 
 struct Work {
   int dp_tiles, rem_tiles, split;
+  unsigned* tickets = nullptr;
 };
 
 __device__ __forceinline__ int xcd_remap(int b, int n) {
@@ -159,6 +160,7 @@
 struct WorkItem {
   int tile, kb, ke, pslot;
 };
+
 
 __device__ __forceinline__ WorkItem get_work(int b, const Work& wk, int nk) {
   WorkItem it;
@@ -197,6 +199,93 @@
     for (int j = 0; j < TN; ++j)
 #pragma unroll
       for (int e = 0; e < 16; ++e) acc[i][j][e] = 0.f;
+}
+
+template <int TM, int TN, int NT>
+__device__ __forceinline__ void store_partial_wt(float* __restrict__ slab, int pslot, const f32x16 (&acc)[TM][TN], int tid) {
+  constexpr int SEG = TM * TN * 16 * NT * 4;
+  const __amdgpu_buffer_rsrc_t sr = __builtin_amdgcn_make_buffer_rsrc((void*)(slab + (size_t)pslot * (SEG / 4)), 0, SEG, 0x00020000);
+#pragma unroll
+  for (int i = 0; i < TM; ++i)
+#pragma unroll
+    for (int j = 0; j < TN; ++j)
+#pragma unroll
+      for (int q = 0; q < 4; ++q) {
+        u32x4 d;
+        d.x = __float_as_uint(acc[i][j][4 * q]);
+        d.y = __float_as_uint(acc[i][j][4 * q + 1]);
+        d.z = __float_as_uint(acc[i][j][4 * q + 2]);
+        d.w = __float_as_uint(acc[i][j][4 * q + 3]);
+        __builtin_amdgcn_raw_buffer_store_b128(d, sr, (((i * TN + j) * 4 + q) * NT + tid) * 16, 0, 16);
+      }
+}
+
+template <int TM, int TN, int NT>
+__device__ __forceinline__ void sum_partials_wt(const float* __restrict__ slab, int rt, int split, int own, f32x16 (&acc)[TM][TN], int tid) {
+  constexpr int SEG = TM * TN * 16 * NT * 4;
+  constexpr int U = 4;
+  const __amdgpu_buffer_rsrc_t sr =
+      __builtin_amdgcn_make_buffer_rsrc((void*)(slab + (size_t)rt * split * (SEG / 4)), 0, split * SEG, 0x00020000);
+#pragma unroll
+  for (int i = 0; i < TM; ++i)
+#pragma unroll
+    for (int j = 0; j < TN; ++j) {
+      const int voff = ((i * TN + j) * 4 * NT + tid) * 16;
+      auto add_range = [&](f32x16& d, int sb, int se) __attribute__((always_inline)) {
+        for (int s0 = sb; s0 < se; s0 += U) {
+          u32x4 v[U][4];
+#pragma unroll
+          for (int u = 0; u < U; ++u)
+#pragma unroll
+            for (int q = 0; q < 4; ++q)
+              v[u][q] = __builtin_amdgcn_raw_buffer_load_b128(sr, (voff + q * NT * 16) | (s0 + u < se ? 0 : kOOB), (s0 + u) * SEG, 16);
+#pragma unroll
+          for (int u = 0; u < U; ++u)
+#pragma unroll
+            for (int q = 0; q < 4; ++q) {
+              d[4 * q] += __uint_as_float(v[u][q].x);
+              d[4 * q + 1] += __uint_as_float(v[u][q].y);
+              d[4 * q + 2] += __uint_as_float(v[u][q].z);
+              d[4 * q + 3] += __uint_as_float(v[u][q].w);
+            }
+        }
+      };
+      f32x16 t;
+#pragma unroll
+      for (int e = 0; e < 16; ++e) t[e] = 0.f;
+      add_range(t, 0, own);
+#pragma unroll
+      for (int e = 0; e < 16; ++e) acc[i][j][e] = t[e] + acc[i][j][e];
+      add_range(acc[i][j], own + 1, split);
+    }
+}
+
+template <int TM, int TN, int NT, bool ACQ>
+__device__ __forceinline__ bool ksplit_last_arriver(float* __restrict__ slab, const Work& wk, int pslot, f32x16 (&acc)[TM][TN],
+                                                    unsigned* flag, int tid) {
+  const int rt = pslot / wk.split;
+  store_partial_wt<TM, TN, NT>(slab, pslot, acc, tid);
+  if (wk.tickets == nullptr) return false;
+  asm volatile("s_waitcnt vmcnt(0)" ::: "memory");
+  __syncthreads();
+  if (tid == 0) {
+    const unsigned t = __hip_atomic_fetch_add(wk.tickets + rt, 1u, __ATOMIC_RELAXED, __HIP_MEMORY_SCOPE_AGENT);
+    const bool last = t == (unsigned)(wk.split - 1);
+    if (last) {
+      __hip_atomic_store(wk.tickets + rt, 0u, __ATOMIC_RELAXED, __HIP_MEMORY_SCOPE_AGENT);
+      if (ACQ) {
+        __builtin_amdgcn_fence(__ATOMIC_ACQUIRE, "agent");
+        asm volatile("s_waitcnt vmcnt(0)" ::: "memory");
+      }
+    }
+    *flag = last ? 1u : 0u;
+  }
+  __syncthreads();
+  __builtin_amdgcn_fence(__ATOMIC_ACQUIRE, "wavefront");
+  if (*flag == 0u) return false;
+  __syncthreads();
+  sum_partials_wt<TM, TN, NT>(slab, rt, wk.split, pslot - rt * wk.split, acc, tid);
+  return true;
 }
 
 __device__ __forceinline__ void fprop_store(float* __restrict__ y, const Geom& g, int row, int col, float v) {
@@ -999,7 +1088,7 @@
   fprop_epilogue<BM, BN, WM, WN>(acc, smem, y, g, epi, mt, nt, tid);
 }
 
-template <int BM, int BN, int WM, int WN>
+template <int BM, int BN, int WM, int WN, bool WT = false>
 __global__ __launch_bounds__(64 * WM * WN) void conv_fprop_fixup_kernel(const float* __restrict__ slab, float* __restrict__ y, Geom g,
                                                                 int NT, Work wk, FpropEpi epi) {
   constexpr int TM = BM / WM / 32, TN = BN / WN / 32;
@@ -1018,7 +1107,8 @@
 #pragma unroll
       for (int j = 0; j < TN; ++j)
 #pragma unroll
-        for (int e = 0; e < 16; ++e) acc[i][j][e] += src[(size_t)((i * TN + j) * 16 + e) * NTHR];
+        for (int e = 0; e < 16; ++e)
+          acc[i][j][e] += WT ? src[(size_t)(((i * TN + j) * 4 + e / 4) * NTHR) * 4 + 3 * tid + e % 4] : src[(size_t)((i * TN + j) * 16 + e) * NTHR];
   }
   fprop_epilogue<BM, BN, WM, WN>(acc, smem, y, g, epi, mt, nt, tid);
 }
@@ -1300,7 +1390,7 @@
   });
 }
 
-template <int BM, int BN, int WM, int WN>
+template <int BM, int BN, int WM, int WN, bool WT = false>
 __global__ __launch_bounds__(64 * WM * WN) void conv_dgrad_fixup_kernel(const float* __restrict__ slab, float* __restrict__ dx,
                                                                 const float* __restrict__ add_src,
                                                                 const uint32_t* __restrict__ add_mask, Geom g, int NT, Work wk,
@@ -1321,7 +1411,8 @@
 #pragma unroll
       for (int j = 0; j < TN; ++j)
 #pragma unroll
-        for (int e = 0; e < 16; ++e) acc[i][j][e] += src[(size_t)((i * TN + j) * 16 + e) * NTHR];
+        for (int e = 0; e < 16; ++e)
+          acc[i][j][e] += WT ? src[(size_t)(((i * TN + j) * 4 + e / 4) * NTHR) * 4 + 3 * tid + e % 4] : src[(size_t)((i * TN + j) * 16 + e) * NTHR];
   }
   dgrad_epilogue<BM, BN, WM, WN>(acc, smem, tid, dx, add_src, add_mask, g, mt, nt, g.M, stat, [](int mrow) { return mrow; });
 }
@@ -1860,6 +1951,13 @@
 
 constexpr int pl_waves_per_simd(int waves, int np, bool fits128) { return np == 1 && waves == 8 && fits128 ? 4 : waves == 4 ? 2 : waves / 4; }
 
+constexpr bool pl_fprop_inkernel(int BM, int BN, int waves, int NP, bool PRE, int ES) {
+  return ES == 4 && !PRE && pl_waves_per_simd(waves, NP, BN == 64 || (BM == 128 && BN == 256)) < 4 && !(BM == 128 && BN == 256 && NP == 3);
+}
+constexpr bool pl_dgrad_inkernel(int BM, int BN, int waves, int NP, int ES) {
+  return ES == 4 && BM != 64 && pl_waves_per_simd(waves, NP, BN == 64) < 4;
+}
+
 template <int BM, int BN, int WM, int WN, int NBUF, int NP = 3, bool PRE = false, int ES = 4>
 __global__ __launch_bounds__(64 * WM * WN, pl_waves_per_simd(WM * WN, NP, BN == 64 || (BM == 128 && BN == 256))) void conv_fprop_pl_kernel(const void* __restrict__ x,
                                                                                       const unsigned short* __restrict__ wp,
@@ -2002,11 +2100,22 @@
   }
   BDV_STAMP(2);
 
-  if (it.pslot >= 0) {
-    store_partial<TM, TN, NTHR>(slab, it.pslot, acc, tid);
+  if constexpr (!pl_fprop_inkernel(BM, BN, WM * WN, NP, PRE, ES)) {
+    if (it.pslot >= 0) {
+      store_partial<TM, TN, NTHR>(slab, it.pslot, acc, tid);
+      return;
+    }
+  } else if (it.pslot >= 0) {
+    constexpr bool ACQ = pl_waves_per_simd(WM * WN, NP, BN == 64 || (BM == 128 && BN == 256)) * 4 > WM * WN;
+    int tid2 = tid;
+    asm volatile("" : "+v"(tid2));
+    if (!ksplit_last_arriver<TM, TN, NTHR, ACQ>(slab, wk, it.pslot, acc, reinterpret_cast<unsigned*>(smem_b), tid2)) return;
+    fprop_epilogue<BM, BN, WM, WN, ES>(acc, smem, y, g, epi, mt, nt, tid2);
     return;
   }
-  fprop_epilogue<BM, BN, WM, WN, ES>(acc, smem, y, g, epi, mt, nt, tid);
+  int tid3 = tid;
+  asm volatile("" : "+v"(tid3));
+  fprop_epilogue<BM, BN, WM, WN, ES>(acc, smem, y, g, epi, mt, nt, tid3);
   BDV_STAMP(3);
   BDV_STAMP(4);
 }
@@ -2164,12 +2273,24 @@
     }
   }
   BDV_STAMP(2);
-  if (it.pslot >= 0) {
-    store_partial<TM, TN, NTHR>(slab, it.pslot, acc, tid);
+  if constexpr (!pl_dgrad_inkernel(BM, BN, WM * WN, NP, ES)) {
+    if (it.pslot >= 0) {
+      store_partial<TM, TN, NTHR>(slab, it.pslot, acc, tid);
+      return;
+    }
+  } else if (it.pslot >= 0) {
+    constexpr bool ACQ = (BM == 64 ? 4 : pl_waves_per_simd(WM * WN, NP, BN == 64)) * 4 > WM * WN;
+    int tid2 = tid;
+    asm volatile("" : "+v"(tid2));
+    if (!ksplit_last_arriver<TM, TN, NTHR, ACQ>(slab, wk, it.pslot, acc, reinterpret_cast<unsigned*>(smem_b), tid2)) return;
+    dgrad_epilogue<BM, BN, WM, WN, true, ES, TM * TN <= 4 && NP >= 2 && BM != 64>(acc, smem, tid2, dx, add_src, add_mask, g, mt, nt, Mc, stat,
+                                                                                [](int mrow) { return mrow; });
     return;
   }
   constexpr bool EPI_PIPE = TM * TN <= 4 && NP >= 2 && BM != 64;
-  dgrad_epilogue<BM, BN, WM, WN, true, ES, EPI_PIPE>(acc, smem, tid, dx, add_src, add_mask, g, mt, nt, Mc, stat, [&](int mrow) {
+  int tid3 = tid;
+  asm volatile("" : "+v"(tid3));
+  dgrad_epilogue<BM, BN, WM, WN, true, ES, EPI_PIPE>(acc, smem, tid3, dx, add_src, add_mask, g, mt, nt, Mc, stat, [&](int mrow) {
     if (st == 1) return mrow;
     const int n = mrow / HcWc;
     const int rem = mrow - n * HcWc;
@@ -2629,6 +2750,22 @@
 int pl_tile_override() {
   if (g_pl_tile_forced == -2) g_pl_tile_forced = getenv("BDVCIL_PL_TILE") ? atoi(getenv("BDVCIL_PL_TILE")) : -1;
   return g_pl_tile_forced;
+}
+
+int g_ksplit_fixup = -2;
+bool ksplit_fixup_forced() {
+  if (g_ksplit_fixup == -2) g_ksplit_fixup = getenv("BDVCIL_KSPLIT_FIXUP") != nullptr && atoi(getenv("BDVCIL_KSPLIT_FIXUP")) != 0 ? 1 : 0;
+  return g_ksplit_fixup == 1;
+}
+constexpr int kTicketWords = 512;
+
+int g_last_pl_plan[5] = {-1, 0, 0, 1, 0};
+void record_pl_plan(int cfg, const Work& wk) {
+  g_last_pl_plan[0] = cfg;
+  g_last_pl_plan[1] = wk.dp_tiles;
+  g_last_pl_plan[2] = wk.rem_tiles;
+  g_last_pl_plan[3] = wk.split;
+  g_last_pl_plan[4] = wk.split > 1 && wk.tickets != nullptr ? 1 : 0;
 }
 
 int pl_pick(bool dgrad, int ncols, int nk, int taps, int stride, int pieces = 3, bool shifted = false) {
@@ -3034,6 +3171,41 @@
   return BDV_OK;
 }
 
+extern "C" int bdv_conv_debug_force_fixup(int on) {
+  BDV_REQUIRE(on >= -1 && on <= 1, "bdv_conv_debug_force_fixup: %d (1 = fix-up launch, 0 = in-kernel combine, -1 = BDVCIL_KSPLIT_FIXUP)", on);
+  g_ksplit_fixup = on < 0 ? -2 : on;
+  return BDV_OK;
+}
+
+extern "C" size_t bdv_conv_ksplit_ticket_bytes(void) { return kTicketWords * sizeof(unsigned); }
+
+extern "C" int bdv_conv_debug_pl_plan(const bdv_conv_geom* gg, int kind, int pieces, int* out5) {
+  if (int e = check_geom(gg, "bdv_conv_debug_pl_plan")) return e;
+  BDV_REQUIRE(out5 != nullptr && (kind == 0 || kind == 1) && pieces >= 1 && pieces <= 3, "bdv_conv_debug_pl_plan: bad argument");
+  const int cfg = kind == 0 ? pl_fprop_cfg(gg, pieces) : pl_dgrad_cfg(gg, pieces);
+  out5[0] = cfg;
+  out5[1] = out5[2] = out5[4] = 0;
+  out5[3] = 1;
+  if (cfg < 0) return BDV_OK;
+  const bool split_ok = gg->act_dtype != BDV_ACT_BF16 && (kind == 0 || gg->stride == 1);
+  const PlPlan p = kind == 0 ? plan_pl(cfg, gg->N * gg->Ho * gg->Wo, gg->Cout, gg->R * gg->S * gg->Cin / BK, kMaxSplitWorkspace, split_ok)
+                             : plan_pl(cfg, gg->N * gg->H * gg->W, gg->Cin, gg->R * gg->S * gg->Cout / BK, kMaxSplitWorkspace, split_ok);
+  const int waves = pl_cfg_wm(cfg) * pl_cfg_wn(cfg);
+  const bool ink = kind == 0 ? pl_fprop_inkernel(kPlCfg[cfg].BM, kPlCfg[cfg].BN, waves, pieces, false, 4)
+                             : pl_dgrad_inkernel(kPlCfg[cfg].BM, kPlCfg[cfg].BN, waves, pieces, 4);
+  out5[1] = p.wk.dp_tiles;
+  out5[2] = p.wk.rem_tiles;
+  out5[3] = p.wk.split;
+  out5[4] = ink && p.wk.split > 1 && !ksplit_fixup_forced() && p.wk.rem_tiles <= kTicketWords ? 1 : 0;
+  return BDV_OK;
+}
+
+extern "C" int bdv_conv_debug_last_plan(int* out5) {
+  BDV_REQUIRE(out5 != nullptr, "bdv_conv_debug_last_plan: null pointer");
+  for (int i = 0; i < 5; ++i) out5[i] = g_last_pl_plan[i];
+  return BDV_OK;
+}
+
 extern "C" int bdv_conv_kernel_name(const bdv_conv_geom* gg, int kind, int arith, char* out, size_t n) {
   if (int e = check_geom(gg, "bdv_conv_kernel_name")) return e;
   BDV_REQUIRE(out && n > 0 && kind >= 0 && kind <= 2, "bdv_conv_kernel_name: bad argument");
@@ -3120,10 +3292,14 @@
   return pl_fprop_cfg_pre(gg) >= 0 && gg->fold == 0 ? 1 : 0;
 }
 
-extern "C" int bdv_conv_fprop_pl(const void* x, const float* w, const void* planes_fprop, void* y, const bdv_conv_geom* gg,
-                                 float* bn_partial, const bdv_conv_affine* affine, void* workspace, size_t workspace_bytes,
-                                 int pieces, const float* pre_scale, const float* pre_shift, void* stream) {
+namespace {
+int conv_fprop_pl_impl(const void* x, const float* w, const void* planes_fprop, void* y, const bdv_conv_geom* gg,
+                       float* bn_partial, const bdv_conv_affine* affine, void* workspace, size_t workspace_bytes,
+                       int pieces, const float* pre_scale, const float* pre_shift, unsigned* tickets, size_t tickets_bytes,
+                       void* stream) {
   if (int e = check_geom(gg, "bdv_conv_fprop_pl")) return e;
+  BDV_REQUIRE(tickets == nullptr || (tickets_bytes >= kTicketWords * sizeof(unsigned) && ((uintptr_t)tickets & 3) == 0),
+              "bdv_conv_fprop_pl_tickets: tickets need bdv_conv_ksplit_ticket_bytes() = %zu bytes (got %zu)", kTicketWords * sizeof(unsigned), tickets_bytes);
   BDV_REQUIRE(pieces >= 1 && pieces <= 3, "bdv_conv_fprop_pl: pieces = %d (3, 2 or 1)", pieces);
   const bool pre = pre_scale != nullptr;
   const bool h16 = gg->act_dtype == BDV_ACT_BF16;
@@ -3136,9 +3312,11 @@
                 "bdv_conv_fprop_pl: a producer BatchNorm in the loader needs the plane kernels (pieces 3, no temporal shift, Cin %% 32 == 0)");
     BDV_REQUIRE(bdv_aligned16(pre_scale) && bdv_aligned16(pre_shift), "bdv_conv_fprop_pl: pre_scale / pre_shift must be 16-byte aligned");
   }
-  if (!pre && (planes_fprop == nullptr || !pl_fprop_ok(gg, pieces)))
+  if (!pre && (planes_fprop == nullptr || !pl_fprop_ok(gg, pieces))) {
+    record_pl_plan(-1, Work{0, 0, 1});
     return conv_fprop_impl((const float*)x, w, (float*)y, gg, bn_partial, affine, workspace, workspace_bytes, stream, true,
                            gg->Cin % BK == 0 && r1_planes_enabled() ? planes_fprop : nullptr);
+  }
   BDV_REQUIRE(x && y, "bdv_conv_fprop_pl: null pointer");
   FpropEpi epi = {bn_partial, 0, nullptr, nullptr, nullptr, 0, pre_scale, pre_shift};
   if (affine != nullptr) {
@@ -3158,8 +3336,11 @@
   g.Ktot = g.Rt * g.R * g.S * g.Cin;
   BDV_REQUIRE((int64_t)3 * g.Cout * g.Ktot * 2 < (1ll << 31), "bdv_conv_fprop_pl: weight planes exceed 2^31 bytes");
   hipStream_t s = (hipStream_t)stream;
-  const PlPlan p = plan_pl(pre ? pl_fprop_cfg_pre(gg) : pl_fprop_cfg(gg, pieces), g.M, g.Cout, g.Ktot / BK, workspace ? (workspace_bytes < kMaxSplitWorkspace ? workspace_bytes : kMaxSplitWorkspace) : 0, !h16);
+  PlPlan p = plan_pl(pre ? pl_fprop_cfg_pre(gg) : pl_fprop_cfg(gg, pieces), g.M, g.Cout, g.Ktot / BK, workspace ? (workspace_bytes < kMaxSplitWorkspace ? workspace_bytes : kMaxSplitWorkspace) : 0, !h16);
   BDV_REQUIRE(p.cfg >= 0, "bdv_conv_fprop_pl: no tile configuration for Cout=%d", g.Cout);
+  const bool ink = pl_fprop_inkernel(kPlCfg[p.cfg].BM, kPlCfg[p.cfg].BN, pl_cfg_wm(p.cfg) * pl_cfg_wn(p.cfg), pre ? 3 : pieces, pre, h16 ? 2 : 4);
+  if (ink && p.wk.split > 1 && tickets != nullptr && !ksplit_fixup_forced() && p.wk.rem_tiles <= kTicketWords) p.wk.tickets = tickets;
+  record_pl_plan(p.cfg, p.wk);
   const int blocks = p.wk.dp_tiles + p.wk.rem_tiles * p.wk.split;
   epi.MT = p.MT;
   float* slab = (float*)workspace;
@@ -3185,9 +3366,13 @@
       hipLaunchKernelGGL((conv_fprop_pl_kernel<BM_, BN_, WM_, WN_, NB_, 3>), dim3(blocks), dim3(64 * WM_ * WN_), 0, s, x, wp, y, g,    \
                          p.NT, p.wk, slab, epi);                                                                                      \
     BDV_LAUNCH_CHECK("bdv_conv_fprop_pl");                                                                                            \
-    if (p.wk.split > 1) {                                                                                                             \
-      hipLaunchKernelGGL((conv_fprop_fixup_kernel<BM_, BN_, WM_, WN_>), dim3(p.wk.rem_tiles), dim3(64 * WM_ * WN_), 0, s,             \
-                         (const float*)slab, (float*)y, g, p.NT, p.wk, epi);                                                                  \
+    if (p.wk.split > 1 && p.wk.tickets == nullptr) {                                                                                  \
+      if (ink)                                                                                                                        \
+        hipLaunchKernelGGL((conv_fprop_fixup_kernel<BM_, BN_, WM_, WN_, true>), dim3(p.wk.rem_tiles), dim3(64 * WM_ * WN_), 0, s,     \
+                           (const float*)slab, (float*)y, g, p.NT, p.wk, epi);                                                        \
+      else                                                                                                                            \
+        hipLaunchKernelGGL((conv_fprop_fixup_kernel<BM_, BN_, WM_, WN_>), dim3(p.wk.rem_tiles), dim3(64 * WM_ * WN_), 0, s,           \
+                           (const float*)slab, (float*)y, g, p.NT, p.wk, epi);                                                        \
       BDV_LAUNCH_CHECK("bdv_conv_fprop_pl(fixup)");                                                                                   \
     }                                                                                                                                 \
   } while (0)
@@ -3199,20 +3384,41 @@
 #undef BDV_FPROP_PL
   return BDV_OK;
 }
-
-extern "C" int bdv_conv_dgrad_pl(const void* dy, const float* w, const void* planes_dgrad, void* dx, const void* add_src,
-                                 const uint32_t* add_mask_src, const bdv_conv_geom* gg, const bdv_bn_stat_fuse* bn_stat,
-                                 void* workspace, size_t workspace_bytes, int pieces, void* stream) {
+}
+
+extern "C" int bdv_conv_fprop_pl(const void* x, const float* w, const void* planes_fprop, void* y, const bdv_conv_geom* gg,
+                                 float* bn_partial, const bdv_conv_affine* affine, void* workspace, size_t workspace_bytes,
+                                 int pieces, const float* pre_scale, const float* pre_shift, void* stream) {
+  return conv_fprop_pl_impl(x, w, planes_fprop, y, gg, bn_partial, affine, workspace, workspace_bytes, pieces, pre_scale, pre_shift,
+                            nullptr, 0, stream);
+}
+
+extern "C" int bdv_conv_fprop_pl_tickets(const void* x, const float* w, const void* planes_fprop, void* y, const bdv_conv_geom* gg,
+                                         float* bn_partial, const bdv_conv_affine* affine, void* workspace, size_t workspace_bytes,
+                                         int pieces, const float* pre_scale, const float* pre_shift, void* tickets,
+                                         size_t tickets_bytes, void* stream) {
+  return conv_fprop_pl_impl(x, w, planes_fprop, y, gg, bn_partial, affine, workspace, workspace_bytes, pieces, pre_scale, pre_shift,
+                            (unsigned*)tickets, tickets_bytes, stream);
+}
+
+namespace {
+int conv_dgrad_pl_impl(const void* dy, const float* w, const void* planes_dgrad, void* dx, const void* add_src,
+                       const uint32_t* add_mask_src, const bdv_conv_geom* gg, const bdv_bn_stat_fuse* bn_stat,
+                       void* workspace, size_t workspace_bytes, int pieces, unsigned* tickets, size_t tickets_bytes, void* stream) {
   if (int e = check_geom(gg, "bdv_conv_dgrad_pl")) return e;
+  BDV_REQUIRE(tickets == nullptr || (tickets_bytes >= kTicketWords * sizeof(unsigned) && ((uintptr_t)tickets & 3) == 0),
+              "bdv_conv_dgrad_pl_tickets: tickets need bdv_conv_ksplit_ticket_bytes() = %zu bytes (got %zu)", kTicketWords * sizeof(unsigned), tickets_bytes);
   BDV_REQUIRE(pieces >= 1 && pieces <= 3, "bdv_conv_dgrad_pl: pieces = %d (3, 2 or 1)", pieces);
   const bool h16 = gg->act_dtype == BDV_ACT_BF16;
   BDV_REQUIRE_ACT(gg->act_dtype, "bdv_conv_dgrad_pl");
   if (h16)
     BDV_REQUIRE(pieces == 1 && planes_dgrad != nullptr && pl_dgrad_ok(gg, 1),
                 "bdv_conv_dgrad_pl: bf16 activation storage needs pieces = 1, the weight planes, Cout %% 32 == 0 and Cin %% 64 == 0 (Cin=%d Cout=%d)", gg->Cin, gg->Cout);
-  if (planes_dgrad == nullptr || !pl_dgrad_ok(gg, pieces))
+  if (planes_dgrad == nullptr || !pl_dgrad_ok(gg, pieces)) {
+    record_pl_plan(-1, Work{0, 0, 1});
     return conv_dgrad_impl((const float*)dy, w, nullptr, (float*)dx, (const float*)add_src, add_mask_src, gg, bn_stat, workspace, workspace_bytes, stream,
                            gg->Cout % BK == 0 && r1_planes_enabled() ? planes_dgrad : nullptr);
+  }
   BnStat stat = {nullptr, nullptr, nullptr, nullptr, nullptr, 0, nullptr, nullptr};
   if (bn_stat != nullptr) {
     BDV_REQUIRE(gg->stride == 1 || (gg->R >= gg->stride && gg->S >= gg->stride),
@@ -3244,6 +3450,9 @@
                      workspace ? (workspace_bytes < kMaxSplitWorkspace ? workspace_bytes : kMaxSplitWorkspace) : 0, st == 1 && !h16);
   BDV_REQUIRE(p.cfg >= 0, "bdv_conv_dgrad_pl: no tile configuration for Cin=%d", g.Cin);
   if (st != 1) p.wk.dp_tiles = ((p.MT + 7) / 8) * 8 * p.NT;
+  const bool ink = pl_dgrad_inkernel(kPlCfg[p.cfg].BM, kPlCfg[p.cfg].BN, pl_cfg_wm(p.cfg) * pl_cfg_wn(p.cfg), pieces, h16 ? 2 : 4);
+  if (ink && p.wk.split > 1 && tickets != nullptr && !ksplit_fixup_forced() && p.wk.rem_tiles <= kTicketWords) p.wk.tickets = tickets;
+  record_pl_plan(p.cfg, p.wk);
   stat.MT = st * st * p.MT;
   if (st != 1 && stat.y != nullptr)
     (void)hipMemsetAsync(stat.partial, 0, (size_t)2 * stat.MT * g.Cin * sizeof(float), s);
@@ -3269,9 +3478,13 @@
       hipLaunchKernelGGL((conv_dgrad_pl_kernel<BM_, BN_, WM_, WN_, NB_, 3>), grid, dim3(64 * WM_ * WN_), 0, s, dy, dp, dx, add_src,     \
                          add_mask_src, g, p.NT, p.wk, slab, stat);                                                                     \
     BDV_LAUNCH_CHECK("bdv_conv_dgrad_pl");                                                                                             \
-    if (p.wk.split > 1) {                                                                                                              \
-      hipLaunchKernelGGL((conv_dgrad_fixup_kernel<BM_, BN_, WM_, WN_>), dim3(p.wk.rem_tiles), dim3(64 * WM_ * WN_), 0, s,              \
-                         (const float*)slab, (float*)dx, (const float*)add_src, add_mask_src, g, p.NT, p.wk, stat);                                          \
+    if (p.wk.split > 1 && p.wk.tickets == nullptr) {                                                                                   \
+      if (ink)                                                                                                                         \
+        hipLaunchKernelGGL((conv_dgrad_fixup_kernel<BM_, BN_, WM_, WN_, true>), dim3(p.wk.rem_tiles), dim3(64 * WM_ * WN_), 0, s,      \
+                           (const float*)slab, (float*)dx, (const float*)add_src, add_mask_src, g, p.NT, p.wk, stat);                  \
+      else                                                                                                                             \
+        hipLaunchKernelGGL((conv_dgrad_fixup_kernel<BM_, BN_, WM_, WN_>), dim3(p.wk.rem_tiles), dim3(64 * WM_ * WN_), 0, s,            \
+                           (const float*)slab, (float*)dx, (const float*)add_src, add_mask_src, g, p.NT, p.wk, stat);                  \
       BDV_LAUNCH_CHECK("bdv_conv_dgrad_pl(fixup)");                                                                                    \
     }                                                                                                                                  \
   } while (0)
@@ -3283,6 +3496,22 @@
   else BDV_DGRAD_PL(256, 64, 4, 2, 2);
 #undef BDV_DGRAD_PL
   return BDV_OK;
+}
+}
+
+extern "C" int bdv_conv_dgrad_pl(const void* dy, const float* w, const void* planes_dgrad, void* dx, const void* add_src,
+                                 const uint32_t* add_mask_src, const bdv_conv_geom* gg, const bdv_bn_stat_fuse* bn_stat,
+                                 void* workspace, size_t workspace_bytes, int pieces, void* stream) {
+  return conv_dgrad_pl_impl(dy, w, planes_dgrad, dx, add_src, add_mask_src, gg, bn_stat, workspace, workspace_bytes, pieces, nullptr, 0,
+                            stream);
+}
+
+extern "C" int bdv_conv_dgrad_pl_tickets(const void* dy, const float* w, const void* planes_dgrad, void* dx, const void* add_src,
+                                         const uint32_t* add_mask_src, const bdv_conv_geom* gg, const bdv_bn_stat_fuse* bn_stat,
+                                         void* workspace, size_t workspace_bytes, int pieces, void* tickets, size_t tickets_bytes,
+                                         void* stream) {
+  return conv_dgrad_pl_impl(dy, w, planes_dgrad, dx, add_src, add_mask_src, gg, bn_stat, workspace, workspace_bytes, pieces,
+                            (unsigned*)tickets, tickets_bytes, stream);
 }
 
 namespace {
diff --git a/background-debiased-video-cil_amd/kernels.py b/background-debiased-video-cil_amd/kernels.py
--- a/background-debiased-video-cil_amd/kernels.py
+++ b/background-debiased-video-cil_amd/kernels.py
@@ -103,6 +103,19 @@
     if need == 0:
         check(-1, 'bdv_conv_workspace_bytes')
     return workspace(need, device, tag + WS_TAG_SUFFIX)
+
+
+_CONV_TICKETS = {}
+
+
+def _conv_tickets(device, tag: str) -> torch.Tensor:
+    dev = torch.device(device)
+    key = (dev.index or 0, tag + WS_TAG_SUFFIX, torch.cuda.current_stream(dev).cuda_stream)
+    cur = _CONV_TICKETS.get(key)
+    if cur is None:
+        cur = torch.zeros(lib().bdv_conv_ksplit_ticket_bytes(), dtype=torch.uint8, device=dev)
+        _CONV_TICKETS[key] = cur
+    return cur
 
 
 import os as _os
@@ -294,10 +307,12 @@
         aff = ConvAffine(scale.data_ptr(), shift.data_ptr(), res.data_ptr() if res is not None else None, int(bool(relu)))
     if use_pl:
         planes_f, _ = weight_planes(w, g)
-        check(lib().bdv_conv_fprop_pl(_p(x), _p(w), _p(planes_f), _p(y), ctypes.byref(g), _p(part),
-                                      ctypes.byref(aff) if aff is not None else None, _p(ws), ws.numel(), PIECES,
-                                      _p(pre_bn[0] if pre_bn is not None else None), _p(pre_bn[1] if pre_bn is not None else None),
-                                      _stream()), 'bdv_conv_fprop_pl')
+        tk = _conv_tickets(x.device, ws_tag)
+        check(lib().bdv_conv_fprop_pl_tickets(_p(x), _p(w), _p(planes_f), _p(y), ctypes.byref(g), _p(part),
+                                              ctypes.byref(aff) if aff is not None else None, _p(ws), ws.numel(), PIECES,
+                                              _p(pre_bn[0] if pre_bn is not None else None),
+                                              _p(pre_bn[1] if pre_bn is not None else None), _p(tk), tk.numel(), _stream()),
+              'bdv_conv_fprop_pl_tickets')
         return (y, part) if bn_stats else y
     fn = lib().bdv_conv_fprop_x3 if use_x3 else lib().bdv_conv_fprop
     check(fn(_p(x), _p(w), _p(y), ctypes.byref(g), _p(part), ctypes.byref(aff) if aff is not None else None,
@@ -353,9 +368,11 @@
     ws = _conv_ws(g, 1, dy.device, ws_tag)
     if use_pl:
         _, planes_d = weight_planes(w, g)
-        check(lib().bdv_conv_dgrad_pl(_p(dy), _p(w), _p(planes_d), _p(dx), _p(add_src), _p(add_mask_src), ctypes.byref(g),
-                                      ctypes.byref(fuse) if fuse is not None else None, _p(ws), ws.numel(), PIECES, _stream()),
-              'bdv_conv_dgrad_pl')
+        tk = _conv_tickets(dy.device, ws_tag)
+        check(lib().bdv_conv_dgrad_pl_tickets(_p(dy), _p(w), _p(planes_d), _p(dx), _p(add_src), _p(add_mask_src), ctypes.byref(g),
+                                              ctypes.byref(fuse) if fuse is not None else None, _p(ws), ws.numel(), PIECES,
+                                              _p(tk), tk.numel(), _stream()),
+              'bdv_conv_dgrad_pl_tickets')
         return dx if bn_stats is None else (dx, partial)
     if use_x3 and g.Cin % 128 == 0:
         w_t = w.permute(1, 2, 3, 0).contiguous()
diff --git a/include/bdvcil_hip.h b/include/bdvcil_hip.h
--- a/include/bdvcil_hip.h
+++ b/include/bdvcil_hip.h
@@ -82,6 +82,16 @@
 int bdv_conv_dgrad_pl(const void* dy, const float* w, const void* planes_dgrad, void* dx, const void* add_src,
                       const uint32_t* add_mask_src, const bdv_conv_geom* g, const bdv_bn_stat_fuse* bn_stat, void* workspace,
                       size_t workspace_bytes, int pieces, void* stream);
+size_t bdv_conv_ksplit_ticket_bytes(void);
+int bdv_conv_fprop_pl_tickets(const void* x, const float* w, const void* planes_fprop, void* y, const bdv_conv_geom* g,
+                              float* bn_partial, const bdv_conv_affine* affine, void* workspace, size_t workspace_bytes, int pieces,
+                              const float* pre_scale, const float* pre_shift, void* tickets, size_t tickets_bytes, void* stream);
+int bdv_conv_dgrad_pl_tickets(const void* dy, const float* w, const void* planes_dgrad, void* dx, const void* add_src,
+                              const uint32_t* add_mask_src, const bdv_conv_geom* g, const bdv_bn_stat_fuse* bn_stat, void* workspace,
+                              size_t workspace_bytes, int pieces, void* tickets, size_t tickets_bytes, void* stream);
+int bdv_conv_debug_force_fixup(int on);
+int bdv_conv_debug_last_plan(int* out5);
+int bdv_conv_debug_pl_plan(const bdv_conv_geom* g, int kind, int pieces, int* out5);
 
 int bdv_conv_wgrad(const float* dy, const float* x, float* dw, float beta, const bdv_conv_geom* g, void* workspace,
                    size_t workspace_bytes, void* stream);
```

Result: no change. 608.3 clips/s (median of 2 runs) (-0.1%).
